# citibeth/spsparse

Hardware: NVIDIA B200
Metric: spgemm_intermediate_products_per_sec (higher is better)
Workload: dtype f64

## Files before the change

### spsparse_b200/csrc/radix_sort.cuh

```cuda
#pragma once
#include "common.cuh"

constexpr int RS_THREADS = 256;
#ifndef RS_IPT_N
#define RS_IPT_N 16
#endif
#ifndef RS_MIN_BLOCKS
#define RS_MIN_BLOCKS 3
#endif
constexpr int RS_IPT = RS_IPT_N;
constexpr int RS_HB = RS_IPT / 2;
constexpr int RS_TILE = RS_THREADS * RS_IPT;
constexpr int RS_WARPS = RS_THREADS / 32;
constexpr int RS_RADIX_BITS = 8;
constexpr int RS_RADIX = 1 << RS_RADIX_BITS;
constexpr int RS_NB = RS_RADIX + 1;
constexpr int RS_MAX_PASSES = 8;
#ifndef RS_LOOKBACK
#define RS_LOOKBACK 8
#endif
constexpr size_t RS_SMEM_BYTES =
    (size_t)RS_TILE * 16 + (size_t)RS_WARPS * RS_NB * sizeof(u32) + 64;

#define RS_WORD_AGG(c) ((c) + 1u)
// ... 72 lines not shown
    constexpr int HU = 4;
    for (u64 i0 = (u64)blockIdx.x * blockDim.x + threadIdx.x; i0 < in.n; i0 += HU * stride) {
        i32 hi[HU], lo[HU];
        double v[HU];
#pragma unroll
        for (int u = 0; u < HU; ++u) {
            const u64 i = i0 + u * stride;
            const u64 ic = i < in.n ? i : i0;
            hi[u] = ld_stream_i32(in.hi + ic);
            lo[u] = in.lo ? ld_stream_i32(in.lo + ic) : 0;
            v[u] = ld_stream_f64(in.val + ic);
        }
#pragma unroll
        for (int u = 0; u < HU; ++u) {
            const u64 i = i0 + u * stride;
            if (i >= in.n) break;
            if ((u32)hi[u] >= in.extent_hi || (u32)lo[u] >= in.extent_lo) { oob = 1; continue; }
            if (!input_kept(in, (u32)i, v[u])) continue;
            ++kept;
            u64 key = pack_key(hi[u], lo[u], in.bits_lo) >> shift0;
            for (int p = 0; p < passes; ++p) {
                atomicAdd(&s_h[p * RS_RADIX + (u32)(key & (RS_RADIX - 1))], 1u);
                key >>= RS_RADIX_BITS;
            }
        }
    }
    __syncthreads();
    for (int t = threadIdx.x; t < passes * RS_RADIX; t += blockDim.x)
        if (s_h[t]) atomicAdd(&hist[t], s_h[t]);
#pragma unroll
    for (int o = 16; o > 0; o >>= 1) kept += __shfl_xor_sync(SPB_FULL_MASK, kept, o);
    if (lane_id() == 0 && kept) atomicAdd(&counters[0], kept);
    if (oob) counters[1] = 1;
}

__global__ void __launch_bounds__(512) k_keys_hist(const u64 *__restrict__ keys, u64 n, int passes, u32 *hist) {
    __shared__ u32 s_h[RS_MAX_PASSES * RS_RADIX];
    for (int t = threadIdx.x; t < passes * RS_RADIX; t += blockDim.x) s_h[t] = 0;
    __syncthreads();
    const u64 stride = (u64)gridDim.x * blockDim.x;
    for (u64 i = (u64)blockIdx.x * blockDim.x + threadIdx.x; i < n; i += stride) {
        u64 key = ld_stream_u64(keys + i);
        for (int p = 0; p < passes; ++p) {
            atomicAdd(&s_h[p * RS_RADIX + (u32)(key & (RS_RADIX - 1))], 1u);
            key >>= RS_RADIX_BITS;
        }
    }
    __syncthreads();
    for (int t = threadIdx.x; t < passes * RS_RADIX; t += blockDim.x)
        if (s_h[t]) atomicAdd(&hist[t], s_h[t]);
}

__global__ void __launch_bounds__(RS_RADIX) k_bucket_starts(u32 *hist) {
    __shared__ u32 s_w[RS_RADIX / 32];
    u32 *h = hist + blockIdx.x * RS_RADIX;
    u32 c = h[threadIdx.x];
    u32 incl = warp_incl_scan(c);
    if (lane_id() == 31) s_w[threadIdx.x >> 5] = incl;
    __syncthreads();
    u32 add = 0;
    for (u32 w = 0; w < (threadIdx.x >> 5); ++w) add += s_w[w];
    h[threadIdx.x] = add + incl - c;
}

struct PassArgs {
    const u64 *keys_in;
    const double *vals_in;
    u64 *keys_out;
    double *vals_out;
    const u32 *n_ptr;
    const u32 *bucket_start;
    u32 *lookback;
    u32 *ticket;
    int shift;
    int rank_mode;
};

template <bool PASS0, bool BULK = false>
__global__ void __launch_bounds__(RS_THREADS, RS_MIN_BLOCKS) k_radix_pass(PassArgs a, SortInput in) {
    __shared__ __align__(8) u64 s_mbar[2];
    extern __shared__ __align__(128) unsigned char smem_raw[];
    u64 *s_keys = reinterpret_cast<u64 *>(smem_raw);
    double *s_vals = reinterpret_cast<double *>(s_keys + RS_TILE);
    u32 *s_wcnt = reinterpret_cast<u32 *>(s_vals + RS_TILE);
    u32 *s_misc = s_wcnt + RS_WARPS * RS_NB;

    const u32 tid = threadIdx.x, lane = tid & 31, warp = tid >> 5;
    if (tid == 0) {
        s_misc[0] = atomicAdd(a.ticket, 1u);
        if (BULK) { mbar_init(&s_mbar[0], 1); mbar_init(&s_mbar[1], 1); mbar_fence_init(); }
    }
    for (int t = tid; t < RS_WARPS * RS_NB; t += RS_THREADS) s_wcnt[t] = 0;
    __syncthreads();
    const u32 tile = s_misc[0];
    const u32 n = PASS0 ? in.n : *a.n_ptr;
    const u64 tile_base = (u64)tile * RS_TILE;
    if (tile_base >= n) return;
    if (BULK && PASS0 && tid == 0) {
        i32 *s_idx = reinterpret_cast<i32 *>(s_keys);
        mbar_expect_tx(&s_mbar[0], (in.lo ? 2u : 1u) * RS_TILE * 4u);
        bulk_load(s_idx, in.hi + tile_base, RS_TILE * 4u, &s_mbar[0]);
        if (in.lo) bulk_load(s_idx + RS_TILE, in.lo + tile_base, RS_TILE * 4u, &s_mbar[0]);
        mbar_expect_tx(&s_mbar[1], RS_TILE * 8u);
        bulk_load(s_vals, in.val + tile_base, RS_TILE * 8u, &s_mbar[1]);
    }
    if (BULK && !PASS0 && tid == 0) {
        const u32 valid = n - tile_base < (u64)RS_TILE ? (u32)(n - tile_base) : (u32)RS_TILE;
        const u32 bytes = (valid * 8u + 15u) & ~15u;
        mbar_expect_tx(&s_mbar[0], bytes);
        bulk_load(s_keys, a.keys_in + tile_base, bytes, &s_mbar[0]);
        mbar_expect_tx(&s_mbar[1], bytes);
        bulk_load(s_vals, a.vals_in + tile_base, bytes, &s_mbar[1]);
    }

    const u64 wbase = tile_base + (u64)warp * (32 * RS_IPT) + lane;
    u64 key[RS_IPT];
    u32 valid_bits = 0;
    if (PASS0 && BULK) {
        mbar_wait(&s_mbar[0], 0);
        mbar_wait(&s_mbar[1], 0);
        const i32 *s_idx = reinterpret_cast<const i32 *>(s_keys);
#pragma unroll
        for (int k = 0; k < RS_IPT; ++k) {
            const u32 q = warp * (32 * RS_IPT) + k * 32 + lane;
            const i32 hi = s_idx[q], lo = in.lo ? s_idx[RS_TILE + q] : 0;
            const bool ok = ((u32)hi < in.extent_hi) && ((u32)lo < in.extent_lo) && input_kept(in, (u32)(tile_base + q), s_vals[q]);
            key[k] = pack_key(hi, lo, in.bits_lo);
            valid_bits |= (ok ? 1u : 0u) << k;
        }
    } else if (PASS0) {
#pragma unroll
        for (int h = 0; h < RS_IPT; h += RS_HB) {
            i32 hi[RS_HB], lo[RS_HB];
            double v[RS_HB];
#pragma unroll
            for (int k = 0; k < RS_HB; ++k) {
                u64 i = wbase + (u64)(h + k) * 32;
                u64 ic = i < n ? i : (u64)n - 1;
                hi[k] = ld_stream_i32(in.hi + ic);
                lo[k] = in.lo ? ld_stream_i32(in.lo + ic) : 0;
                v[k] = in.val[ic];
            }
#pragma unroll
            for (int k = 0; k < RS_HB; ++k) {
                u64 i = wbase + (u64)(h + k) * 32;
                bool ok = (i < n) && ((u32)hi[k] < in.extent_hi) && ((u32)lo[k] < in.extent_lo) &&
                          input_kept(in, (u32)i, v[k]);
                key[h + k] = pack_key(hi[k], lo[k], in.bits_lo);
                valid_bits |= (ok ? 1u : 0u) << (h + k);
            }
        }
    } else if (BULK) {
        mbar_wait(&s_mbar[0], 0);
#pragma unroll
        for (int k = 0; k < RS_IPT; ++k) {
            const bool ok = wbase + (u64)k * 32 < n;
            key[k] = ok ? s_keys[warp * (32 * RS_IPT) + k * 32 + lane] : 0;
            valid_bits |= (ok ? 1u : 0u) << k;
        }
    } else {
#pragma unroll
        for (int k = 0; k < RS_IPT; ++k) {
            u64 i = wbase + (u64)k * 32;
            bool ok = i < n;
            key[k] = ok ? ld_stream_u64(a.keys_in + i) : 0;
            valid_bits |= (ok ? 1u : 0u) << k;
        }
#pragma unroll
        for (int k = 0; k < RS_IPT; ++k) {
            u64 i = wbase + (u64)k * 32;
            if (i < n && (lane & 15) == 0) asm volatile("prefetch.global.L2 [%0];" ::"l"(a.vals_in + i));
        }
    }

    u32 *mycnt = s_wcnt + warp * RS_NB;
    const u32 lt = lanemask_lt();
    unsigned short pos[RS_IPT];
#pragma unroll
    for (int k = 0; k < RS_IPT; ++k) {
        const bool ok = (valid_bits >> k) & 1u;
        const u32 d = (u32)((key[k] >> a.shift) & (RS_RADIX - 1));
        u32 peers;
        if (a.rank_mode == 0) {
            peers = __ballot_sync(SPB_FULL_MASK, ok);
#pragma unroll
            for (int b = 0; b < RS_RADIX_BITS; ++b) {
                int sgn;
                asm("bfe.s32 %0, %1, %2, 1;" : "=r"(sgn) : "r"(d), "r"(b));
                const u32 m = __ballot_sync(SPB_FULL_MASK, sgn != 0);
                peers &= ~(m ^ (u32)sgn);
            }
        } else {
            peers = __match_any_sync(SPB_FULL_MASK, ok ? d : (u32)RS_RADIX);
        }
        u32 leader = ok ? (u32)(__ffs(peers) - 1) : lane;
        u32 before = 0;
        if (ok && lane == leader) {
            before = mycnt[d];
            mycnt[d] = before + __popc(peers);
        }
        before = __shfl_sync(SPB_FULL_MASK, before, leader);
        pos[k] = (unsigned short)(before + __popc(peers & lt));
        __syncwarp();
    }
    __syncthreads();

    u32 total = 0;
#pragma unroll
    for (int w = 0; w < RS_WARPS; ++w) total += s_wcnt[w * RS_NB + tid];
    u32 *lb = a.lookback + (u64)tile * RS_RADIX + tid;
    st_relaxed_u32(lb, tile == 0 ? RS_WORD_INCL(total) : RS_WORD_AGG(total));
    u32 incl = warp_incl_scan(total);
    if (lane == 31) s_misc[1 + warp] = incl;
    __syncthreads();
    u32 lstart = incl - total;
    for (u32 w = 0; w < warp; ++w) lstart += s_misc[1 + w];
    const u32 nvalid_if_last = lstart + total;
    {
        u32 run = lstart;
#pragma unroll
        for (int w = 0; w < RS_WARPS; ++w) {
            u32 c = s_wcnt[w * RS_NB + tid];
            s_wcnt[w * RS_NB + tid] = run;
            run += c;
        }
    }
    if (tid == RS_RADIX - 1) s_misc[12] = nvalid_if_last;
    __syncthreads();
    const u32 nvalid = s_misc[12];

#pragma unroll
    for (int k = 0; k < RS_IPT; ++k) {
        if ((valid_bits >> k) & 1u) {
            u32 d = (u32)((key[k] >> a.shift) & (RS_RADIX - 1));
            u32 p = mycnt[d] + pos[k];
            pos[k] = (unsigned short)p;
            s_keys[p] = key[k];
        }
    }
    {
        const double *vsrc = PASS0 ? in.val : a.vals_in;
        double v[RS_IPT];
        if (BULK) {
            mbar_wait(&s_mbar[1], 0);
#pragma unroll
            for (int k = 0; k < RS_IPT; ++k) v[k] = s_vals[warp * (32 * RS_IPT) + k * 32 + lane];
            __syncthreads();
        } else {
#pragma unroll
            for (int k = 0; k < RS_IPT; ++k) {
                u64 i = wbase + (u64)k * 32;
                v[k] = ((valid_bits >> k) & 1u) ? ld_stream_f64(vsrc + i) : 0.0;
            }
        }
#pragma unroll
        for (int k = 0; k < RS_IPT; ++k)
            if ((valid_bits >> k) & 1u) s_vals[pos[k]] = v[k];
    }

    u32 excl = 0;
    if (tile > 0) {
        i64 p = (i64)tile - 1;
        bool done = false;
        while (!done) {
            u32 w[RS_LOOKBACK];
#pragma unroll
            for (int u = 0; u < RS_LOOKBACK; ++u)
                w[u] = (p - u >= 0) ? ld_relaxed_u32(a.lookback + (u64)(p - u) * RS_RADIX + tid) : RS_WORD_INCL(0u);
#pragma unroll
            for (int u = 0; u < RS_LOOKBACK; ++u) {
                if (done) break;
                while (!RS_READY(w[u])) w[u] = ld_relaxed_u32(a.lookback + (u64)(p - u) * RS_RADIX + tid);
                excl += RS_VALUE(w[u]);
                if (RS_IS_INCL(w[u])) done = true;
            }
            p -= RS_LOOKBACK;
        }
        st_relaxed_u32(lb, RS_WORD_INCL(excl + total));
    }
    const u32 gbase = a.bucket_start[tid] + excl - lstart;
    __syncthreads();
    s_wcnt[tid] = gbase;
    __syncthreads();

#pragma unroll
    for (int k = 0; k < RS_IPT; ++k) {
        u32 p = (u32)k * RS_THREADS + tid;
        if (p < nvalid) {
            u64 kk = s_keys[p];
            u32 dst = s_wcnt[(u32)((kk >> a.shift) & (RS_RADIX - 1))] + p;
            a.keys_out[dst] = kk;
            a.vals_out[dst] = s_vals[p];
        }
    }
}

constexpr int SG_THREADS = 256;
constexpr int SG_IPT = 8;
constexpr int SG_TILE = SG_THREADS * SG_IPT;
constexpr int SEG_MAX = 64;

constexpr int SG_CNT_SHIFT = 8;
__global__ void __launch_bounds__(SG_THREADS, 5) k_segment_sort(const u64 *__restrict__ keys_in, const double *__restrict__ vals_in,
                                                                const u32 *n_ptr, int bits_lo, u64 *keys_out, double *vals_out,
                                                                unsigned char *flags, u32 *long_count, u64 *tile_cnt = nullptr,
                                                                int keep_all = 0) {
    constexpr int W = SG_TILE + 2 * SEG_MAX;
    constexpr int ITS = (W + SG_THREADS - 1) / SG_THREADS;
    constexpr int NG = ITS * SG_THREADS / 32;
    __shared__ u64 s_key[W];
    __shared__ u32 s_col[W];
    __shared__ u32 s_hb[NG];
    __shared__ u32 s_last[NG];
    __shared__ u32 s_first[NG];
    const u32 n = *n_ptr;
    const u64 base = (u64)blockIdx.x * SG_TILE;
    if (base >= n) return;
    const u32 tid = threadIdx.x, lane = tid & 31, warp = tid >> 5;
    for (u32 q = tid; q < (u32)W; q += SG_THREADS) {
        const i64 g = (i64)base + (i64)q - SEG_MAX;
        s_key[q] = (g >= 0 && g < (i64)n) ? ld_stream_u64(keys_in + g) : ~0ull;
    }
#pragma unroll
    for (int k = 0; k < SG_IPT; ++k) {
        const u64 g = base + (u64)warp * 256 + (u64)k * 32 + lane;
        if (g < n && (lane & 15) == 0) asm volatile("prefetch.global.L2 [%0];" ::"l"(vals_in + g));
    }
    __syncthreads();
    const u64 lo_mask = (1ull << bits_lo) - 1;
#pragma unroll
    for (int it = 0; it < ITS; ++it) {
        const u32 q = (u32)it * SG_THREADS + tid;
        bool head = true;
        if (q < (u32)W) {
            const u64 kk = s_key[q];
            s_col[q] = (u32)(kk & lo_mask);
            head = q == 0 || (s_key[q - 1] >> bits_lo) != (kk >> bits_lo);
        }
        const u32 hb = __ballot_sync(SPB_FULL_MASK, head);
        if (lane == 0) {
            const u32 g = q >> 5;
            s_hb[g] = hb;
            s_last[g] = hb ? (g << 5) + 31 - __clz(hb) : 0;
            s_first[g] = hb ? (g << 5) + __ffs(hb) - 1 : 0xffffffffu;
        }
    }
    __syncthreads();
    if (warp == 0) {
        u32 carry = 0;
        for (int r = 0; r < (NG + 31) / 32; ++r) {
            const int g = r * 32 + (int)lane;
            const u32 mine = g < NG ? s_last[g] : 0;
            u32 inc = mine;
#pragma unroll
            for (int o = 1; o < 32; o <<= 1) {
                const u32 t = __shfl_up_sync(SPB_FULL_MASK, inc, o);
                if (lane >= (u32)o) inc = max(inc, t);
            }
            u32 exc = __shfl_up_sync(SPB_FULL_MASK, inc, 1);
            if (lane == 0) exc = 0;
            if (g < NG) s_last[g] = max(exc, carry);
            carry = max(carry, __shfl_sync(SPB_FULL_MASK, inc, 31));
        }
        carry = 0xffffffffu;
        for (int r = (NG + 31) / 32 - 1; r >= 0; --r) {
            const int g = r * 32 + (int)lane;
            const u32 mine = g < NG ? s_first[g] : 0xffffffffu;
            u32 inc = mine;
#pragma unroll
            for (int o = 1; o < 32; o <<= 1) {
                const u32 t = __shfl_down_sync(SPB_FULL_MASK, inc, o);
                if (lane + o < 32) inc = min(inc, t);
            }
            u32 exc = __shfl_down_sync(SPB_FULL_MASK, inc, 1);
            if (lane == 31) exc = 0xffffffffu;
            if (g < NG) s_first[g] = min(exc, carry);
            carry = min(carry, __shfl_sync(SPB_FULL_MASK, inc, 0));
        }
    }
    __syncthreads();
    u32 n_long = 0;
    i32 shift_by[SG_IPT];
    u32 cnt_at = 0, cnt_before = 0, cnt_after = 0;
    const u64 wbase = base + (u64)warp * 256;
#pragma unroll
    for (int k = 0; k < SG_IPT; ++k) {
        const u32 q = SEG_MAX + warp * 256 + (u32)k * 32 + lane;
        const u64 g = wbase + (u64)k * 32 + lane;
        shift_by[k] = 0;
        if (g < n) {
            bool head = true, rhead = false;
            const u32 grp = q >> 5, l = q & 31, hb = s_hb[grp];
            const u32 below = hb & (0xffffffffu >> (31 - l));
            const u32 st = below ? (grp << 5) + 31 - __clz(below) : s_last[grp];
            const u32 above = l < 31 ? hb & (0xffffffffu << (l + 1)) : 0u;
            const u32 nx = above ? (grp << 5) + __ffs(above) - 1 : s_first[grp];
            const bool is_long = nx - st > (u32)SEG_MAX;
            if (!is_long) {
                const u32 col = s_col[q];
                u32 before = 0, same = 0;
                for (u32 j = st; j < q; ++j) { before += s_col[j] <= col; same += s_col[j] == col; }
                for (u32 j = q + 1; j < nx; ++j) before += s_col[j] < col;
                shift_by[k] = (i32)(st + before) - (i32)q;
                head = keep_all || same == 0;
                rhead = before == 0;
            }
            if (flags) flags[g] = is_long;
            n_long += is_long;
            const u64 dst = (u64)((i64)g + shift_by[k]);
            const u32 inc = (head ? 1u : 0u) | (rhead ? 0x10000u : 0u);
            if (dst < wbase) cnt_before += inc;
            else if (dst >= wbase + 256) cnt_after += inc;
            else cnt_at += inc;
        }
    }
    if (tile_cnt) {
        const u32 a0 = __reduce_add_sync(SPB_FULL_MASK, cnt_at), a1 = __reduce_add_sync(SPB_FULL_MASK, cnt_before),
                  a2 = __reduce_add_sync(SPB_FULL_MASK, cnt_after);
        if (lane == 0) {
            u64 *t = tile_cnt + (wbase >> SG_CNT_SHIFT);
            if (a0) atomicAdd((ull *)t, (ull)(a0 & 0xffffu) | ((ull)(a0 >> 16) << 31));
            if (a1) atomicAdd((ull *)(t - 1), (ull)(a1 & 0xffffu) | ((ull)(a1 >> 16) << 31));
            if (a2) atomicAdd((ull *)(t + 1), (ull)(a2 & 0xffffu) | ((ull)(a2 >> 16) << 31));
        }
    }
    double v[SG_IPT];
#pragma unroll
    for (int k = 0; k < SG_IPT; ++k) {
        const u64 g = wbase + (u64)k * 32 + lane;
        v[k] = g < n ? ld_stream_f64(vals_in + g) : 0.0;
    }
#pragma unroll
    for (int k = 0; k < SG_IPT; ++k) {
        const u64 g = wbase + (u64)k * 32 + lane;
        if (g < n) {
            const u64 dst = (u64)((i64)g + shift_by[k]);
            keys_out[dst] = s_key[SEG_MAX + warp * 256 + k * 32 + lane];
            vals_out[dst] = v[k];
        }
    }
    n_long = __reduce_add_sync(SPB_FULL_MASK, n_long);
    if (n_long && lane == 0) atomicAdd(long_count, n_long);
}

static_assert(SG_TILE % 256 == 0 && (1 << SG_CNT_SHIFT) == 256, "a warp's 256 consecutive entries are one tile of the reduce pass");
#ifndef SGW_UNROLL_N
#define SGW_UNROLL_N 8
#endif
constexpr int SGW_UNROLL = SGW_UNROLL_N;
__global__ void __launch_bounds__(SG_THREADS, 6) k_segment_sort_walk(const u64 *__restrict__ keys_in, const double *__restrict__ vals_in,
                                                             const u32 *n_ptr, int bits_lo, u64 *keys_out, double *vals_out,
                                                             unsigned char *flags, u32 *long_count, u64 *tile_cnt = nullptr,
                                                             int keep_all = 0) {
    __shared__ u32 s_row[SG_TILE + 2 * SEG_MAX];
    __shared__ u32 s_col[SG_TILE + 2 * SEG_MAX];
    const u32 n = *n_ptr;
    const u64 base = (u64)blockIdx.x * SG_TILE;
    if (base >= n) return;
    const u32 tid = threadIdx.x;
    const u32 lo_mask = bits_lo >= 32 ? 0xffffffffu : (1u << bits_lo) - 1u;
    for (u32 q = tid; q < SG_TILE + 2 * SEG_MAX; q += SG_THREADS) {
        const i64 g = (i64)base + (i64)q - SEG_MAX;
        u32 row = 0xffffffffu, col = 0;
        if (g >= 0 && g < (i64)n) {
            const u64 key = ld_stream_u64(keys_in + g);
            row = (u32)(key >> bits_lo);
            col = (u32)key & lo_mask;
        }
        s_row[q] = row;
        s_col[q] = col;
    }
    const u32 lane = tid & 31, warp = tid >> 5;
    const u64 wbase = base + (u64)warp * 256;
    double v[SG_IPT];
#pragma unroll
    for (int k = 0; k < SG_IPT; ++k) {
        const u64 g = wbase + (u64)k * 32 + lane;
        v[k] = g < n ? ld_stream_f64(vals_in + g) : 0.0;
    }
    __syncthreads();
    u32 n_long = 0;
    u32 cnt_at = 0, cnt_before = 0, cnt_after = 0;
#pragma unroll
    for (int k = 0; k < SG_IPT; ++k) {
        const u32 q = SEG_MAX + warp * 256 + (u32)k * 32 + lane;
        const u64 g = wbase + (u64)k * 32 + lane;
        u64 dst = g;
        bool head = true, rhead = false;
        if (g < n) {
            const u32 row = s_row[q], col = s_col[q];
            u32 b = 0, f = 0, before = 0, same = 0;
            if (s_row[q - SEG_MAX] == row || s_row[q + SEG_MAX] == row) b = f = (u32)SEG_MAX;
            else {
#pragma unroll SGW_UNROLL
                for (b = 0; b < (u32)SEG_MAX; ++b) {
                    if (s_row[q - 1 - b] != row) break;
                    const u32 c = s_col[q - 1 - b];
                    before += c <= col;
                    same += c == col;
                }
#pragma unroll SGW_UNROLL
                for (f = 0; f < (u32)SEG_MAX; ++f) {
                    if (s_row[q + 1 + f] != row) break;
                    before += s_col[q + 1 + f] < col;
                }
            }
            const bool is_long = b == (u32)SEG_MAX || f == (u32)SEG_MAX || b + f + 1 > (u32)SEG_MAX;
            if (!is_long) {
                dst = g - b + before;
                head = keep_all || same == 0;
                rhead = before == 0;
            }
            keys_out[dst] = ((u64)row << bits_lo) | col;
            vals_out[dst] = v[k];
            if (flags) flags[g] = is_long;
            n_long += is_long;
            const u32 inc = (head ? 1u : 0u) | (rhead ? 0x10000u : 0u);
            if (dst < wbase) cnt_before += inc;
            else if (dst >= wbase + 256) cnt_after += inc;
            else cnt_at += inc;
        }
    }
    if (tile_cnt) {
        const u32 a0 = __reduce_add_sync(SPB_FULL_MASK, cnt_at), a1 = __reduce_add_sync(SPB_FULL_MASK, cnt_before),
                  a2 = __reduce_add_sync(SPB_FULL_MASK, cnt_after);
        if (lane == 0) {
            u64 *t = tile_cnt + (wbase >> SG_CNT_SHIFT);
            if (a0) atomicAdd((ull *)t, (ull)(a0 & 0xffffu) | ((ull)(a0 >> 16) << 31));
            if (a1) atomicAdd((ull *)(t - 1), (ull)(a1 & 0xffffu) | ((ull)(a1 >> 16) << 31));
            if (a2) atomicAdd((ull *)(t + 1), (ull)(a2 & 0xffffu) | ((ull)(a2 >> 16) << 31));
        }
    }
    n_long = __reduce_add_sync(SPB_FULL_MASK, n_long);
    if (n_long && lane == 0) atomicAdd(long_count, n_long);
}

constexpr int SGS_ROW = 5;
constexpr int SGS_H = SGS_ROW - 1;
constexpr int SGS_STEP = 32 - 2 * SGS_H;
constexpr int SGS_STEPS = (256 + SGS_STEP - 1) / SGS_STEP;
__global__ void __launch_bounds__(SG_THREADS, 6) k_segment_sort_shfl(const u64 *__restrict__ keys_in, const double *__restrict__ vals_in,
                                                                    const u32 *n_ptr, int bits_lo, u64 *keys_out, double *vals_out,
                                                                    unsigned char *flags, u32 *long_count, u64 *tile_cnt = nullptr,
                                                                    int keep_all = 0) {
    __shared__ u32 s_row[SG_TILE + 2 * SEG_MAX];
    __shared__ u32 s_col[SG_TILE + 2 * SEG_MAX];
    __shared__ double s_val[SG_TILE];
    const u32 n = *n_ptr;
    const u64 base = (u64)blockIdx.x * SG_TILE;
    if (base >= n) return;
    const u32 tid = threadIdx.x, lane = tid & 31, warp = tid >> 5;
    const u32 lo_mask = bits_lo >= 32 ? 0xffffffffu : (1u << bits_lo) - 1u;
    for (u32 q = tid; q < SG_TILE + 2 * SEG_MAX; q += SG_THREADS) {
        const i64 g = (i64)base + (i64)q - SEG_MAX;
        u32 row = 0xffffffffu, col = 0;
        if (g >= 0 && g < (i64)n) {
            const u64 key = ld_stream_u64(keys_in + g);
            row = (u32)(key >> bits_lo);
            col = (u32)key & lo_mask;
        }
        s_row[q] = row;
        s_col[q] = col;
    }
#pragma unroll
    for (int k = 0; k < SG_IPT; ++k) {
        const u32 e = (u32)k * SG_THREADS + tid;
        const u64 g = base + e;
        s_val[e] = g < n ? ld_stream_f64(vals_in + g) : 0.0;
    }
    __syncthreads();
    const u64 wbase = base + (u64)warp * 256;
    u32 n_long = 0;
    u32 cnt_at = 0, cnt_before = 0, cnt_after = 0;
    for (int t = 0; t < SGS_STEPS; ++t) {
        const i32 e = t * SGS_STEP + (i32)lane - SGS_H;
        const u32 q = (u32)(SEG_MAX + (i32)warp * 256 + e);
        const u64 g = wbase + (u64)(i64)e;
        const bool mine = lane >= (u32)SGS_H && lane < (u32)(32 - SGS_H) && e < 256 && g < n;
        const u32 row = s_row[q], col = s_col[q];
        const u32 hb = __ballot_sync(SPB_FULL_MASK, s_row[q - 1] != row);
        const u32 tail = __shfl_sync(SPB_FULL_MASK, (u32)(s_row[q + 1] != row), 31);
        const u64 z = ~((u64)hb | ((u64)tail << 32)) & 0x1ffffffffull;
        u64 run = z;
#pragma unroll
        for (int d = 1; d < SGS_ROW; ++d) run &= z >> d;
        u32 b = 0, f = 0, before = 0, same = 0;
        if (run == 0) {
#pragma unroll
            for (int d = 1; d < SGS_ROW; ++d) {
                const u32 ru = __shfl_up_sync(SPB_FULL_MASK, row, d), cu = __shfl_up_sync(SPB_FULL_MASK, col, d);
                const u32 rd = __shfl_down_sync(SPB_FULL_MASK, row, d), cd = __shfl_down_sync(SPB_FULL_MASK, col, d);
                const bool up = lane >= (u32)d && ru == row, dn = lane + d < 32u && rd == row;
                b += up;
                before += (up && cu <= col) + (dn && cd < col);
                same += up && cu == col;
                f += dn;
            }
        } else if (mine) {
            if (s_row[q - SEG_MAX] == row || s_row[q + SEG_MAX] == row) b = f = (u32)SEG_MAX;
            else {
                for (b = 0; b < (u32)SEG_MAX; ++b) {
                    if (s_row[q - 1 - b] != row) break;
                    const u32 c = s_col[q - 1 - b];
                    before += c <= col;
                    same += c == col;
                }
                for (f = 0; f < (u32)SEG_MAX; ++f) {
                    if (s_row[q + 1 + f] != row) break;
                    before += s_col[q + 1 + f] < col;
                }
            }
        }
        if (mine) {
            const bool is_long = b == (u32)SEG_MAX || f == (u32)SEG_MAX || b + f + 1 > (u32)SEG_MAX;
            u64 dst = g;
            bool head = true, rhead = false;
            if (!is_long) {
                dst = g - b + before;
                head = keep_all || same == 0;
                rhead = before == 0;
            }
            keys_out[dst] = ((u64)row << bits_lo) | col;
            vals_out[dst] = s_val[warp * 256 + (u32)e];
            if (flags) flags[g] = is_long;
            n_long += is_long;
            const u32 inc = (head ? 1u : 0u) | (rhead ? 0x10000u : 0u);
            if (dst < wbase) cnt_before += inc;
            else if (dst >= wbase + 256) cnt_after += inc;
            else cnt_at += inc;
        }
    }
    if (tile_cnt) {
        const u32 a0 = __reduce_add_sync(SPB_FULL_MASK, cnt_at), a1 = __reduce_add_sync(SPB_FULL_MASK, cnt_before),
                  a2 = __reduce_add_sync(SPB_FULL_MASK, cnt_after);
        if (lane == 0) {
            u64 *t = tile_cnt + (wbase >> SG_CNT_SHIFT);
            if (a0) atomicAdd((ull *)t, (ull)(a0 & 0xffffu) | ((ull)(a0 >> 16) << 31));
            if (a1) atomicAdd((ull *)(t - 1), (ull)(a1 & 0xffffu) | ((ull)(a1 >> 16) << 31));
            if (a2) atomicAdd((ull *)(t + 1), (ull)(a2 & 0xffffu) | ((ull)(a2 >> 16) << 31));
        }
    }
    n_long = __reduce_add_sync(SPB_FULL_MASK, n_long);
    if (n_long && lane == 0) atomicAdd(long_count, n_long);
}

__global__ void k_gather_flagged(const u64 *__restrict__ keys, const double *__restrict__ vals, const unsigned char *__restrict__ flags,
                                 const u64 *__restrict__ slot, u32 n, u64 *k_out, double *v_out) {
    for (u64 e = (u64)blockIdx.x * blockDim.x + threadIdx.x; e < n; e += (u64)gridDim.x * blockDim.x)
        if (flags[e]) { k_out[slot[e]] = keys[e]; v_out[slot[e]] = vals[e]; }
}
__global__ void k_scatter_flagged(const u64 *__restrict__ k_sorted, const double *__restrict__ v_sorted,
                                  const unsigned char *__restrict__ flags, const u64 *__restrict__ slot, u32 n, u64 *keys, double *vals) {
    for (u64 e = (u64)blockIdx.x * blockDim.x + threadIdx.x; e < n; e += (u64)gridDim.x * blockDim.x)
        if (flags[e]) { keys[e] = k_sorted[slot[e]]; vals[e] = v_sorted[slot[e]]; }
}
```

### spsparse_b200/csrc/reduce_by_key.cuh

```cuda
#pragma once
#include "scan.cuh"

#ifndef RK_THREADS_N
#define RK_THREADS_N 256
#endif
constexpr int RK_THREADS = RK_THREADS_N;
constexpr int RK_IPT = 8;
constexpr int RK_TILE = RK_THREADS * RK_IPT;
constexpr int RK_WARPS = RK_THREADS / 32;
constexpr u32 RK_LONG_RUN = 256;

enum { POLICY_LEAVE_ALONE = 0, POLICY_ADD = 1, POLICY_REPLACE = 2, POLICY_KEEP_ALL = 3 };
enum { MODE_CONSOLIDATE = 0, MODE_ESC = 1 };

struct ReduceArgs {
    const u64 *keys;
    const double *vals;
    const u32 *n_ptr;
    int bits_lo;
    int policy;
    i32 *out_hi;
    i32 *out_lo;
    double *out_val;
    u32 *out_count;
    u64 *state;
    u32 *ticket;
    u32 *long_list;
    u32 *long_count;
    u32 long_cap;
    u32 *row_start;
    i32 *row_id;
    u32 *row_count;
    const i32 *row_ids;
    i32 row_base;
    const double *si;
    const double *sk;
    double C;
};

__device__ __forceinline__ u32 rk_phys(u32 L) { return L + (L >> 3); }
constexpr int RK_SLOTS = RK_TILE + 2 + ((RK_TILE + 2) >> 3) + 1;

#ifndef RK_MIN_BLOCKS
#define RK_MIN_BLOCKS 5
#endif
template <int MODE>
__global__ void __launch_bounds__(RK_THREADS, RK_MIN_BLOCKS) k_reduce_by_key(ReduceArgs a) {
    __shared__ u64 s_keys[RK_SLOTS];
    __shared__ double s_vals[RK_SLOTS];
    __shared__ u64 s_warp[RK_WARPS];
    __shared__ u32 s_tile;
    __shared__ u64 s_excl;
    const u32 tid = threadIdx.x, lane = tid & 31, warp = tid >> 5;
    const bool want_rows = (MODE == MODE_CONSOLIDATE) && (a.row_start != nullptr);
    if (tid == 0) s_tile = atomicAdd(a.ticket, 1u);
    __syncthreads();
    const u32 tile = s_tile;
    const u32 n = *a.n_ptr;
    const u64 base = (u64)tile * RK_TILE;
    if (base >= n) return;
    const u32 tile_n = (n - base < (u64)RK_TILE) ? (u32)(n - base) : (u32)RK_TILE;

#pragma unroll
    for (int k = 0; k < RK_IPT; ++k) {
        u32 p = (u32)k * RK_THREADS + tid;
        if (p < tile_n) {
            s_keys[rk_phys(p + 1)] = ld_stream_u64(a.keys + base + p);
            s_vals[rk_phys(p + 1)] = ld_stream_f64(a.vals + base + p);
        }
    }
    if (tid == 0) s_keys[0] = base ? a.keys[base - 1] : 0;
    if (tid == 32 && base + RK_TILE < n) s_keys[rk_phys(RK_TILE + 1)] = a.keys[base + RK_TILE];
    __syncthreads();

    const u32 first = tid * RK_IPT;
    const u32 mine = first < tile_n ? (tile_n - first < (u32)RK_IPT ? tile_n - first : (u32)RK_IPT) : 0;
    u64 key[RK_IPT];
    double acc[RK_IPT];
    u32 head_bits = 0, rhead_bits = 0, defer_bits = 0;
    if (mine) {
        u64 prev = s_keys[rk_phys(first)];
#pragma unroll
        for (int j = 0; j < RK_IPT; ++j) {
            key[j] = s_keys[rk_phys(first + j + 1)];
            acc[j] = s_vals[rk_phys(first + j + 1)];
        }
        int cur = -1;
#pragma unroll
        for (int j = 0; j < RK_IPT; ++j) {
            if ((u32)j < mine) {
                const u64 before = j ? key[j - 1] : prev;
                const bool head = (a.policy == POLICY_KEEP_ALL) || (base + first + j == 0) || (key[j] != before);
                if (head) {
                    head_bits |= 1u << j;
                    if (want_rows && ((base + first + j == 0) || (key[j] >> a.bits_lo) != (before >> a.bits_lo)))
                        rhead_bits |= 1u << j;
                    cur = j;
                } else if (cur >= 0) {
                    double v = acc[j];
#pragma unroll
                    for (int h = 0; h < RK_IPT; ++h)
                        if (h == cur) {
                            if (a.policy == POLICY_ADD) acc[h] = __dadd_rn(acc[h], v);
                            else if (a.policy == POLICY_REPLACE) acc[h] = v;
                        }
                }
            }
        }
        if (cur >= 0 && mine == (u32)RK_IPT && (a.policy == POLICY_ADD || a.policy == POLICY_REPLACE)) {
            const u64 k0 = key[RK_IPT - 1];
            double sum = 0.0;
#pragma unroll
            for (int h = 0; h < RK_IPT; ++h) if (h == cur) sum = acc[h];
            u64 q = base + first + RK_IPT;
            u32 steps = 0;
            while (q < n) {
                const u32 L = (u32)(q - base) + 1;
                u64 kq;
                double vq = 0.0;
                if (L <= (u32)RK_TILE) { kq = s_keys[rk_phys(L)]; vq = s_vals[rk_phys(L)]; }
                else if (L == (u32)RK_TILE + 1) { kq = s_keys[rk_phys(L)]; if (kq == k0) vq = a.vals[q]; }
                else { kq = a.keys[q]; if (kq == k0) vq = a.vals[q]; }
                if (kq != k0) break;
                if (a.policy == POLICY_ADD) sum = __dadd_rn(sum, vq); else sum = vq;
                ++q;
                if (MODE == MODE_CONSOLIDATE && ++steps >= RK_LONG_RUN) { defer_bits |= 1u << cur; break; }
            }
#pragma unroll
            for (int h = 0; h < RK_IPT; ++h) if (h == cur) acc[h] = sum;
        }
    }
    u32 emit_bits = head_bits;
    if (MODE == MODE_ESC) {
        const u64 lo_mask = (1ull << a.bits_lo) - 1;
#pragma unroll
        for (int j = 0; j < RK_IPT; ++j)
            if ((head_bits >> j) & 1u) {
                const u32 kcol = (u32)(key[j] & lo_mask);
                if (acc[j] == 0.0 || (a.sk && a.sk[kcol] == 0.0)) emit_bits &= ~(1u << j);
            }
    }
    const u64 my = (u64)__popc(emit_bits) | ((u64)__popc(rhead_bits) << 32);
    const u64 incl = warp_incl_scan(my);
    if (lane == 31) s_warp[warp] = incl;
    __syncthreads();
    u64 wbefore = 0, total = 0;
#pragma unroll
    for (int w = 0; w < RK_WARPS; ++w) {
        const u64 t = s_warp[w];
        if ((u32)w < warp) wbefore += t;
        total += t;
    }
    const u64 before_me = wbefore + incl - my;
    const u32 tile_out = (u32)(total & 0xffffffffull);
    if (warp == 0) {
        const u64 packed = (total & 0xffffffffull) | ((total >> 32) << 31);
        const u64 excl0 = lookback_exclusive(a.state, tile, packed);
        if (lane == 0) {
            s_excl = excl0;
            if (base + RK_TILE >= n) {
                const u64 fin = excl0 + packed;
                const u32 n_out = (u32)(fin & 0x7fffffffull), n_rows = (u32)(fin >> 31);
                *a.out_count = n_out;
                if (want_rows) { *a.row_count = n_rows; a.row_start[n_rows] = n_out; }
            }
        }
    }
    {
        u32 slot = (u32)(before_me & 0xffffffffull);
#pragma unroll
        for (int j = 0; j < RK_IPT; ++j) {
            if ((emit_bits >> j) & 1u) {
                double v = acc[j];
                if (MODE == MODE_ESC) {
                    const u64 lo_mask = (1ull << a.bits_lo) - 1;
                    const i32 hi = (i32)(key[j] >> a.bits_lo) + a.row_base;
                    v = __dmul_rn(v, a.C);
                    v = __dmul_rn(v, a.si ? a.si[a.row_ids[hi]] : 1.0);
                    v = __dmul_rn(v, a.sk ? a.sk[(u32)(key[j] & lo_mask)] : 1.0);
                }
                s_keys[slot] = key[j];
                s_vals[slot] = v;
                ++slot;
            }
        }
    }
    __syncthreads();
    const u64 excl_rows = s_excl >> 31;
    const u64 excl = s_excl & 0x7fffffffull;
    if (MODE == MODE_CONSOLIDATE && (rhead_bits | defer_bits)) {
        u32 slot = (u32)(before_me & 0xffffffffull);
        u64 rslot = excl_rows + (before_me >> 32);
#pragma unroll
        for (int j = 0; j < RK_IPT; ++j) {
            if ((emit_bits >> j) & 1u) {
                if ((rhead_bits >> j) & 1u) {
                    a.row_start[rslot] = (u32)(excl + slot);
                    a.row_id[rslot] = (i32)(key[j] >> a.bits_lo);
                    ++rslot;
                }
                if ((defer_bits >> j) & 1u) {
                    u32 t = atomicAdd(a.long_count, 1u);
                    if (t < a.long_cap) { a.long_list[2 * t] = (u32)(excl + slot); a.long_list[2 * t + 1] = (u32)(base + first + j); }
                }
                ++slot;
            }
        }
    }
    const u64 lo_mask = (1ull << a.bits_lo) - 1;
    for (u32 t = tid; t < tile_out; t += RK_THREADS) {
        const u64 k = s_keys[t];
        i32 hi = (i32)(k >> a.bits_lo);
        if (MODE == MODE_ESC) hi += a.row_base;
        a.out_hi[excl + t] = hi;
        if (a.out_lo) a.out_lo[excl + t] = (i32)(k & lo_mask);
        a.out_val[excl + t] = s_vals[t];
    }
}

__global__ void __launch_bounds__(256) k_long_runs(ReduceArgs a) {
    const u32 n = *a.n_ptr;
    u32 cnt = *a.long_count;
    if (cnt > a.long_cap) cnt = a.long_cap;
    const u32 lane = lane_id();
    const u32 warps = gridDim.x * (blockDim.x >> 5);
    for (u32 t = blockIdx.x * (blockDim.x >> 5) + (threadIdx.x >> 5); t < cnt; t += warps) {
        const u32 slot = a.long_list[2 * t], start = a.long_list[2 * t + 1];
        const u64 key = a.keys[start];
        u32 lo = start + 1, step = RK_LONG_RUN;
        u32 hi = n;
        for (;;) {
            const u64 probe = (u64)lo + step;
            if (probe >= n) break;
            if (a.keys[probe] > key) { hi = (u32)probe; break; }
            lo = (u32)probe + 1;
            step *= 2;
        }
        while (lo < hi) {
            const u32 mid = lo + (hi - lo) / 2;
            if (a.keys[mid] <= key) lo = mid + 1; else hi = mid;
        }
        const u32 end = lo;
        double r;
        if (a.policy == POLICY_ADD) {
            double sum = 0.0;
            bool first = true;
            u32 i = start;
            double v = (i + lane < end) ? a.vals[i + lane] : 0.0;
            while (i < end) {
                const u32 m = end - i < 32u ? end - i : 32u;
                const u32 inext = i + 32;
                const double vn = (inext < end && inext + lane < end) ? a.vals[inext + lane] : 0.0;
                for (u32 l = 0; l < m; ++l) {
                    const double x = __shfl_sync(SPB_FULL_MASK, v, (int)l);
                    if (first) { sum = x; first = false; }
                    else sum = __dadd_rn(sum, x);
                }
                v = vn;
                i = inext;
            }
            r = sum;
        } else {
            r = (a.policy == POLICY_REPLACE) ? a.vals[end - 1] : a.vals[start];
        }
        if (lane == 0) a.out_val[slot] = r;
    }
}
```

### spsparse_b200/csrc/reduce_segsort.cuh

```cuda
#pragma once
#include "radix_sort.cuh"
#include "reduce_by_key.cuh"

constexpr int RF_H = SEG_MAX;
constexpr int RF_W = RK_TILE + 2 * RF_H;
constexpr int RF_ITS = (RF_W + RK_THREADS - 1) / RK_THREADS;
constexpr int RF_SORTED = RK_TILE + RF_H + 1;
constexpr int RF_SLOTS = RF_SORTED + (RF_SORTED >> 3) + 1;

struct RfSmem {
    u64 raw[RF_W];
    u64 keys[RF_SLOTS];
    double vals[RF_SLOTS];
    u64 warp[RK_WARPS];
    u64 excl;
    u32 tile;
};

__global__ void __launch_bounds__(RK_THREADS, 4) k_reduce_segsort(ReduceArgs a, u32 *seg_long) {
    extern __shared__ __align__(16) unsigned char rf_smem[];
    RfSmem &s = *reinterpret_cast<RfSmem *>(rf_smem);
    const u32 tid = threadIdx.x, lane = tid & 31, warp = tid >> 5;
    const bool want_rows = a.row_start != nullptr;
    if (tid == 0) s.tile = atomicAdd(a.ticket, 1u);
    __syncthreads();
    const u32 tile = s.tile;
    const u32 n = *a.n_ptr;
    const u64 base = (u64)tile * RK_TILE;
    if (base >= n) return;
    const u32 tile_n = (n - base < (u64)RK_TILE) ? (u32)(n - base) : (u32)RK_TILE;

    double v[RF_ITS];
#pragma unroll
    for (int k = 0; k < RF_ITS; ++k) {
        const u32 q = (u32)k * RK_THREADS + tid;
        const i64 g = (i64)base + (i64)q - RF_H;
        const bool in = q < (u32)RF_W && g >= 0 && g < (i64)n;
        if (q < (u32)RF_W) s.raw[q] = in ? ld_stream_u64(a.keys + g) : ~0ull;
        v[k] = in ? ld_stream_f64(a.vals + g) : 0.0;
    }
    __syncthreads();

    const u64 lo_mask = (1ull << a.bits_lo) - 1;
    u32 n_long = 0;
#pragma unroll
    for (int k = 0; k < RF_ITS; ++k) {
        const u32 q = (u32)k * RK_THREADS + tid;
        if (q >= (u32)RF_W) continue;
        const u64 key = s.raw[q];
        if (key == ~0ull) continue;
        const u64 row = key >> a.bits_lo, col = key & lo_mask;
        u32 b = 0, f = 0, before = 0;
        bool cut = false;
        for (; b < (u32)SEG_MAX; ++b) {
            if (q < 1 + b) { cut = true; break; }
            const u64 kk = s.raw[q - 1 - b];
            if ((kk >> a.bits_lo) != row) break;
            before += (kk & lo_mask) <= col;
        }
        for (; f < (u32)SEG_MAX; ++f) {
            if (q + 1 + f >= (u32)RF_W) { cut = true; break; }
            const u64 kk = s.raw[q + 1 + f];
            if ((kk >> a.bits_lo) != row) break;
            before += (kk & lo_mask) < col;
        }
        const bool is_long = b == (u32)SEG_MAX || f == (u32)SEG_MAX || b + f + 1 > (u32)SEG_MAX;
        if (q >= (u32)RF_H && q < (u32)(RF_H + RK_TILE)) n_long += is_long;
        const u32 place = (cut || is_long) ? q : q - b + before;
        if (place + 1 >= (u32)RF_H && place + 1 < (u32)(RF_H + RF_SORTED)) {
            const u32 L = place + 1 - (u32)RF_H;
            s.keys[rk_phys(L)] = key;
            s.vals[rk_phys(L)] = v[k];
        }
    }
    n_long = __reduce_add_sync(SPB_FULL_MASK, n_long);
    if (n_long && lane == 0) atomicAdd(seg_long, n_long);
    __syncthreads();

    const u32 first = tid * RK_IPT;
    const u32 mine = first < tile_n ? (tile_n - first < (u32)RK_IPT ? tile_n - first : (u32)RK_IPT) : 0;
    u64 key[RK_IPT];
    double acc[RK_IPT];
    u32 head_bits = 0, rhead_bits = 0;
    if (mine) {
        const u64 prev = s.keys[rk_phys(first)];
#pragma unroll
        for (int j = 0; j < RK_IPT; ++j) {
            key[j] = s.keys[rk_phys(first + j + 1)];
            acc[j] = s.vals[rk_phys(first + j + 1)];
        }
        int cur = -1;
#pragma unroll
        for (int j = 0; j < RK_IPT; ++j) {
            if ((u32)j < mine) {
                const u64 before = j ? key[j - 1] : prev;
                const bool head = (a.policy == POLICY_KEEP_ALL) || (base + first + j == 0) || (key[j] != before);
                if (head) {
                    head_bits |= 1u << j;
                    if (want_rows && ((base + first + j == 0) || (key[j] >> a.bits_lo) != (before >> a.bits_lo)))
                        rhead_bits |= 1u << j;
                    cur = j;
                } else if (cur >= 0) {
                    const double vj = acc[j];
#pragma unroll
                    for (int h = 0; h < RK_IPT; ++h)
                        if (h == cur) {
                            if (a.policy == POLICY_ADD) acc[h] = __dadd_rn(acc[h], vj);
                            else if (a.policy == POLICY_REPLACE) acc[h] = vj;
                        }
                }
            }
        }
        if (cur >= 0 && mine == (u32)RK_IPT && (a.policy == POLICY_ADD || a.policy == POLICY_REPLACE)) {
            const u64 k0 = key[RK_IPT - 1];
            double sum = 0.0;
#pragma unroll
            for (int h = 0; h < RK_IPT; ++h) if (h == cur) sum = acc[h];
            u64 q = base + first + RK_IPT;
            while (q < n) {
                const u32 L = (u32)(q - base) + 1;
                if (L >= (u32)RF_SORTED) break;
                if (s.keys[rk_phys(L)] != k0) break;
                const double vq = s.vals[rk_phys(L)];
                if (a.policy == POLICY_ADD) sum = __dadd_rn(sum, vq); else sum = vq;
                ++q;
            }
#pragma unroll
            for (int h = 0; h < RK_IPT; ++h) if (h == cur) acc[h] = sum;
        }
    }
    const u32 emit_bits = head_bits;
    const u64 my = (u64)__popc(emit_bits) | ((u64)__popc(rhead_bits) << 32);
    const u64 incl = warp_incl_scan(my);
    if (lane == 31) s.warp[warp] = incl;
    __syncthreads();
    u64 wbefore = 0, total = 0;
#pragma unroll
    for (int w = 0; w < RK_WARPS; ++w) {
        const u64 t = s.warp[w];
        if ((u32)w < warp) wbefore += t;
        total += t;
    }
    const u64 before_me = wbefore + incl - my;
    const u32 tile_out = (u32)(total & 0xffffffffull);
    if (warp == 0) {
        const u64 packed = (total & 0xffffffffull) | ((total >> 32) << 31);
        const u64 excl0 = lookback_exclusive(a.state, tile, packed);
        if (lane == 0) {
            s.excl = excl0;
            if (base + RK_TILE >= n) {
                const u64 fin = excl0 + packed;
                const u32 n_out = (u32)(fin & 0x7fffffffull), n_rows = (u32)(fin >> 31);
                *a.out_count = n_out;
                if (want_rows) { *a.row_count = n_rows; a.row_start[n_rows] = n_out; }
            }
        }
    }
    {
        u32 slot = (u32)(before_me & 0xffffffffull);
#pragma unroll
        for (int j = 0; j < RK_IPT; ++j) {
            if ((emit_bits >> j) & 1u) {
                s.keys[slot] = key[j];
                s.vals[slot] = acc[j];
                ++slot;
            }
        }
    }
    __syncthreads();
    const u64 excl_rows = s.excl >> 31;
    const u64 excl = s.excl & 0x7fffffffull;
    if (rhead_bits) {
        u32 slot = (u32)(before_me & 0xffffffffull);
        u64 rslot = excl_rows + (before_me >> 32);
#pragma unroll
        for (int j = 0; j < RK_IPT; ++j) {
            if ((emit_bits >> j) & 1u) {
                if ((rhead_bits >> j) & 1u) {
                    a.row_start[rslot] = (u32)(excl + slot);
                    a.row_id[rslot] = (i32)(key[j] >> a.bits_lo);
                    ++rslot;
                }
                ++slot;
            }
        }
    }
    for (u32 t = tid; t < tile_out; t += RK_THREADS) {
        const u64 k = s.keys[t];
        a.out_hi[excl + t] = (i32)(k >> a.bits_lo);
        if (a.out_lo) a.out_lo[excl + t] = (i32)(k & lo_mask);
        a.out_val[excl + t] = s.vals[t];
    }
}
```

### spsparse_b200/csrc/reduce_warp.cuh

```cuda
#pragma once
#include "reduce_by_key.cuh"

constexpr int RW_IPT = 8;
constexpr int RW_TILE = 32 * RW_IPT;
constexpr int RW_WARPS = 8;
constexpr int RW_THREADS = 32 * RW_WARPS;
constexpr int RW_SLOTS = RW_TILE + (RW_TILE >> 3) + 1;
#ifndef RW_MIN_BLOCKS
#define RW_MIN_BLOCKS 4
#endif

template <bool LOOKBACK>
__global__ void __launch_bounds__(RW_THREADS, RW_MIN_BLOCKS) k_reduce_warp(ReduceArgs a) {
    __shared__ u64 s_keys[RW_WARPS][RW_SLOTS];
    __shared__ double s_vals[RW_WARPS][RW_SLOTS];
    __shared__ u32 s_ticket;
    const u32 tid = threadIdx.x, lane = tid & 31, warp = tid >> 5;
    u32 tile = blockIdx.x * RW_WARPS + warp;
    if (LOOKBACK) {
        if (tid == 0) s_ticket = atomicAdd(a.ticket, 1u);
        __syncthreads();
        tile = s_ticket * RW_WARPS + warp;
    }
    const u32 n = *a.n_ptr;
    const u64 base = (u64)tile * RW_TILE;
    if (base >= n) return;
    const u32 tile_n = (n - base < (u64)RW_TILE) ? (u32)(n - base) : (u32)RW_TILE;
    const bool want_rows = a.row_start != nullptr;
    const u32 first = lane * RW_IPT;
    const u32 mine = first < tile_n ? (tile_n - first < (u32)RW_IPT ? tile_n - first : (u32)RW_IPT) : 0;

    u64 key[RW_IPT];
    double acc[RW_IPT];
    if (tile_n == (u32)RW_TILE && ((((uintptr_t)a.keys) | ((uintptr_t)a.vals)) & 15u) == 0) {
        const ulonglong2 *kp = reinterpret_cast<const ulonglong2 *>(a.keys + base + first);
        const double2 *vp = reinterpret_cast<const double2 *>(a.vals + base + first);
#pragma unroll
        for (int j = 0; j < RW_IPT / 2; ++j) {
            const ulonglong2 t = __ldg(kp + j);
            key[2 * j] = t.x; key[2 * j + 1] = t.y;
        }
#pragma unroll
        for (int j = 0; j < RW_IPT / 2; ++j) {
            const double2 t = __ldg(vp + j);
            acc[2 * j] = t.x; acc[2 * j + 1] = t.y;
        }
    } else {
#pragma unroll
        for (int j = 0; j < RW_IPT; ++j) {
            key[j] = 0; acc[j] = 0.0;
            if ((u32)j < mine) { key[j] = a.keys[base + first + j]; acc[j] = a.vals[base + first + j]; }
        }
    }
    u64 prev = __shfl_up_sync(SPB_FULL_MASK, key[RW_IPT - 1], 1);
    if (lane == 0) prev = base ? a.keys[base - 1] : 0;
    u64 next = __shfl_down_sync(SPB_FULL_MASK, key[0], 1);
    const bool more = base + first + RW_IPT < n;
    if (lane == 31 && more) next = a.keys[base + RW_TILE];

    u32 head_bits = 0, rhead_bits = 0, defer_bits = 0;
    if (mine) {
        int cur = -1;
#pragma unroll
        for (int j = 0; j < RW_IPT; ++j) {
            if ((u32)j < mine) {
                const u64 before = j ? key[j - 1] : prev;
                const bool head = (a.policy == POLICY_KEEP_ALL) || (base + first + j == 0) || (key[j] != before);
                if (head) {
                    head_bits |= 1u << j;
                    if (want_rows && ((base + first + j == 0) || (key[j] >> a.bits_lo) != (before >> a.bits_lo)))
                        rhead_bits |= 1u << j;
                    cur = j;
                } else if (cur >= 0) {
                    const double v = acc[j];
#pragma unroll
                    for (int h = 0; h < RW_IPT; ++h)
                        if (h == cur) {
                            if (a.policy == POLICY_ADD) acc[h] = __dadd_rn(acc[h], v);
                            else if (a.policy == POLICY_REPLACE) acc[h] = v;
                        }
                }
            }
        }
        if (cur >= 0 && mine == (u32)RW_IPT && more && next == key[RW_IPT - 1] &&
            (a.policy == POLICY_ADD || a.policy == POLICY_REPLACE)) {
            const u64 k0 = key[RW_IPT - 1];
            double sum = 0.0;
#pragma unroll
            for (int h = 0; h < RW_IPT; ++h) if (h == cur) sum = acc[h];
            u64 q = base + first + RW_IPT;
            u32 steps = 0;
            while (q < n) {
                if (a.keys[q] != k0) break;
                const double vq = a.vals[q];
                if (a.policy == POLICY_ADD) sum = __dadd_rn(sum, vq); else sum = vq;
                ++q;
                if (++steps >= RK_LONG_RUN) { defer_bits |= 1u << cur; break; }
            }
#pragma unroll
            for (int h = 0; h < RW_IPT; ++h) if (h == cur) acc[h] = sum;
        }
    }
    const u32 emit_bits = head_bits;
    const u64 my = (u64)__popc(emit_bits) | ((u64)__popc(rhead_bits) << 32);
    const u64 incl = warp_incl_scan(my);
    const u64 total = __shfl_sync(SPB_FULL_MASK, incl, 31);
    const u64 before_me = incl - my;
    const u32 tile_out = (u32)(total & 0xffffffffull);
    const u64 packed = (total & 0xffffffffull) | ((total >> 32) << 31);
    const u64 excl0 = LOOKBACK ? lookback_exclusive(a.state, tile, packed) : a.state[tile];
    if (lane == 0 && base + RW_TILE >= n) {
        const u64 fin = excl0 + packed;
        const u32 n_out = (u32)(fin & 0x7fffffffull), n_rows = (u32)(fin >> 31);
        *a.out_count = n_out;
        if (want_rows) { *a.row_count = n_rows; a.row_start[n_rows] = n_out; }
    }
    const u64 excl_rows = excl0 >> 31;
    const u64 excl = excl0 & 0x7fffffffull;
    u64 *const sk = s_keys[warp];
    double *const sv = s_vals[warp];
    {
        u32 slot = (u32)(before_me & 0xffffffffull);
        u64 rslot = excl_rows + (before_me >> 32);
#pragma unroll
        for (int j = 0; j < RW_IPT; ++j) {
            if ((emit_bits >> j) & 1u) {
                sk[rk_phys(slot)] = key[j];
                sv[rk_phys(slot)] = acc[j];
                if ((rhead_bits >> j) & 1u) {
                    a.row_start[rslot] = (u32)(excl + slot);
                    a.row_id[rslot] = (i32)(key[j] >> a.bits_lo);
                    ++rslot;
                }
                if ((defer_bits >> j) & 1u) {
                    const u32 t = atomicAdd(a.long_count, 1u);
                    if (t < a.long_cap) { a.long_list[2 * t] = (u32)(excl + slot); a.long_list[2 * t + 1] = (u32)(base + first + j); }
                }
                ++slot;
            }
        }
    }
    __syncwarp();
    const u64 lo_mask = (1ull << a.bits_lo) - 1;
    for (u32 t = lane; t < tile_out; t += 32) {
        const u64 k = sk[rk_phys(t)];
        a.out_hi[excl + t] = (i32)(k >> a.bits_lo);
        if (a.out_lo) a.out_lo[excl + t] = (i32)(k & lo_mask);
        a.out_val[excl + t] = sv[rk_phys(t)];
    }
}
```

### spsparse_b200/csrc/spb_api.cu

```cuda
#include "../../include/spsparse_b200.h"

#include <cstdarg>
#include <cstdio>
#include <cstdlib>
#include <cstring>
#include <chrono>
#include <map>
#include <mutex>
#include <thread>
#include <unordered_map>
#include <vector>

#include "common.cuh"
#include "csr.cuh"
#include "gen.cuh"
#include "radix_sort.cuh"
#include "radix_sort9.cuh"
#include "reduce_by_key.cuh"
#include "reduce_segsort.cuh"
#include "reduce_warp.cuh"
#include "scan.cuh"
#include "spgemm.cuh"
#include "dense_ops.cuh"
#include "rowpart.cuh"

thread_local std::string g_last_error;

int spb_fail(int code, const char *fmt, ...) {
    char buf[1024];
    va_list ap;
    va_start(ap, fmt);
    vsnprintf(buf, sizeof buf, fmt, ap);
    va_end(ap);
    g_last_error = buf;
    return code;
}

static inline double now_ms() {
    return std::chrono::duration<double, std::milli>(std::chrono::steady_clock::now().time_since_epoch()).count();
}
static double g_alloc_ms = 0;
static int g_trace = -1;
static inline bool tracing() {
    if (g_trace < 0) g_trace = getenv("SPB_TRACE") ? 1 : 0;
    return g_trace == 1;
}

struct DevPool {
    std::multimap<size_t, void *> free_;
    std::unordered_map<void *, size_t> live_;
    std::mutex mu_;
    size_t cached_bytes = 0;

    static size_t round_up(size_t b) {
        if (b < 512) return 512;
        if (b < (1u << 20)) return (b + 511) & ~(size_t)511;
        return (b + (1u << 20) - 1) & ~(size_t)((1u << 20) - 1);
    }
    cudaError_t alloc(void **out, size_t bytes) {
        std::lock_guard<std::mutex> g(mu_);
        const size_t want = round_up(bytes);
        auto it = free_.lower_bound(want);
        if (it != free_.end() && it->first <= want + (want >= (64u << 20) ? want / 2 : want / 8)) {
            *out = it->second;
            live_[*out] = it->first;
            cached_bytes -= it->first;
            free_.erase(it);
            return cudaSuccess;
        }
        void *p = nullptr;
        cudaError_t e = cudaMalloc(&p, want);
        if (e != cudaSuccess) {
            cudaGetLastError();
            trim_locked();
            e = cudaMalloc(&p, want);
            if (e != cudaSuccess) return e;
        }
        live_[p] = want;
        *out = p;
        return cudaSuccess;
    }
    void release(void *p) {
        if (!p) return;
        std::lock_guard<std::mutex> g(mu_);
        auto it = live_.find(p);
        if (it == live_.end()) return;
        free_.insert({it->second, p});
        cached_bytes += it->second;
        live_.erase(it);
    }
    void trim_locked() {
        cudaDeviceSynchronize();
        for (auto &kv : free_) cudaFree(kv.second);
        free_.clear();
        cached_bytes = 0;
    }
    void destroy() {
        std::lock_guard<std::mutex> g(mu_);
        trim_locked();
        for (auto &kv : live_) cudaFree(kv.first);
        live_.clear();
    }
};

struct spb_ctx {
    int device;
    cudaStream_t stream;
    bool own_stream;
    int sm_count;
    u32 merge_max_products;
    u64 esc_chunk;
    u64 hash_min_products;
    int hash_variant;
    u64 launches;
    bool bulk_load;
    static constexpr int XFER_WORKERS = 8;
    int xfer_workers;
    static constexpr size_t XFER_CHUNK = 16u << 20;
    void *xfer_buf[XFER_WORKERS][2];
    cudaStream_t xfer_stream[XFER_WORKERS];
    cudaEvent_t xfer_ev[XFER_WORKERS][2];
    bool xfer_ready;
    DevPool pool;
};

struct spb_coo {
    int rank;
    u64 shape[2];
    u64 n;
    i32 *idx[2];
    double *val;
    int sort_order[2];
    bool owned;
    u32 *row_start;
    i32 *row_id;
    u32 nrows;
    bool rows_valid;
    u32 *dense_ptr;
    bool dense_ptr_owned;
    u32 *range_ptr;
    u64 range_lo, range_hi;
    u32 max_row_len;
};

struct Scratch {
    spb_ctx *ctx;
    std::vector<void *> ptrs;
    explicit Scratch(spb_ctx *c) : ctx(c) {}
    ~Scratch() { for (void *p : ptrs) ctx->pool.release(p); }
    template <typename T>
    int get(T **out, u64 count) {
        void *p = nullptr;
        size_t bytes = (size_t)(count ? count : 1) * sizeof(T);
        double t0 = tracing() ? now_ms() : 0;
        cudaError_t e = ctx->pool.alloc(&p, bytes);
        if (tracing()) { double dt = now_ms() - t0; g_alloc_ms += dt; if (dt > 1.0) fprintf(stderr, "[spb] pool.alloc(%zu MB) took %.2f ms\n", bytes >> 20, dt); }
        if (e != cudaSuccess) return spb_fail(SPB_ERR_CUDA, "device allocation of %zu bytes failed: %s", bytes, cudaGetErrorString(e));
        ptrs.push_back(p);
        *out = (T *)p;
        return 0;
    }
    template <typename T>
    int zeroed(T **out, u64 count) {
        CKR(get(out, count));
        CK(cudaMemsetAsync(*out, 0, (size_t)(count ? count : 1) * sizeof(T), ctx->stream));
        return 0;
    }
    void release(void *p) {
        for (size_t i = 0; i < ptrs.size(); ++i)
            if (ptrs[i] == p) { ctx->pool.release(p); ptrs.erase(ptrs.begin() + i); return; }
    }
    void keep(void *p) {
        for (size_t i = 0; i < ptrs.size(); ++i)
            if (ptrs[i] == p) { ptrs.erase(ptrs.begin() + i); return; }
    }
};

struct Timer {
    cudaStream_t s;
    std::vector<cudaEvent_t> ev;
    explicit Timer(cudaStream_t st) : s(st) {}
    ~Timer() { for (auto e : ev) cudaEventDestroy(e); }
    int mark() {
        cudaEvent_t e;
        cudaEventCreate(&e);
        cudaEventRecord(e, s);
        ev.push_back(e);
        return (int)ev.size() - 1;
    }
    float ms(int a, int b) {
        float t = 0;
        cudaEventSynchronize(ev[b]);
        cudaEventElapsedTime(&t, ev[a], ev[b]);
        return t;
    }
};

static inline u32 grid_for(u64 n, u32 threads, u32 cap) {
    u64 g = div_up(n ? n : 1, threads);
    return (u32)(g < cap ? g : cap);
}

static bool host_ptr_is_pinned(const void *p) {
    cudaPointerAttributes at;
    if (cudaPointerGetAttributes(&at, p) != cudaSuccess) { cudaGetLastError(); return false; }
    return at.type == cudaMemoryTypeHost || at.type == cudaMemoryTypeManaged;
}

static int xfer_setup(spb_ctx *c) {
    if (c->xfer_ready) return 0;
    {
        int want = getenv("SPB_XFER_WORKERS") ? atoi(getenv("SPB_XFER_WORKERS")) : (int)(std::thread::hardware_concurrency() / 2);
        c->xfer_workers = want < 1 ? 1 : (want > spb_ctx::XFER_WORKERS ? spb_ctx::XFER_WORKERS : want);
    }
    for (int w = 0; w < c->xfer_workers; ++w) {
        CK(cudaStreamCreateWithFlags(&c->xfer_stream[w], cudaStreamNonBlocking));
        for (int b = 0; b < 2; ++b) {
            CK(cudaHostAlloc(&c->xfer_buf[w][b], spb_ctx::XFER_CHUNK, cudaHostAllocDefault));
            CK(cudaEventCreateWithFlags(&c->xfer_ev[w][b], cudaEventDisableTiming));
        }
    }
    c->xfer_ready = true;
    return 0;
}

struct XferJob { void *dev; void *host; size_t bytes; };

static int staged_copy(spb_ctx *c, const XferJob *jobs, int njobs, bool to_device) {
    bool all_pinned = true;
    size_t total = 0;
    for (int j = 0; j < njobs; ++j) { if (jobs[j].bytes) { all_pinned = all_pinned && host_ptr_is_pinned(jobs[j].host); total += jobs[j].bytes; } }
    if (all_pinned || total < (4u << 20)) {
        for (int j = 0; j < njobs; ++j)
            if (jobs[j].bytes)
                CK(cudaMemcpyAsync(to_device ? jobs[j].dev : jobs[j].host, to_device ? jobs[j].host : jobs[j].dev, jobs[j].bytes,
                                   to_device ? cudaMemcpyHostToDevice : cudaMemcpyDeviceToHost, c->stream));
        CK(cudaStreamSynchronize(c->stream));
        return 0;
    }
    CKR(xfer_setup(c));
    struct Chunk { char *dev; char *host; size_t bytes; };
    std::vector<Chunk> chunks;
    for (int j = 0; j < njobs; ++j)
        for (size_t o = 0; o < jobs[j].bytes; o += spb_ctx::XFER_CHUNK)
            chunks.push_back({(char *)jobs[j].dev + o, (char *)jobs[j].host + o, std::min(spb_ctx::XFER_CHUNK, jobs[j].bytes - o)});
    const int NW = c->xfer_workers;
    cudaError_t err[spb_ctx::XFER_WORKERS];
    auto work = [&](int w) {
        cudaError_t e = cudaSetDevice(c->device);
        int b = 0;
        size_t pending_chunk[2] = {(size_t)-1, (size_t)-1};
        for (size_t k = w; k < chunks.size() && e == cudaSuccess; k += (size_t)NW, b ^= 1) {
            const Chunk &ch = chunks[k];
            if (to_device) {
                e = cudaEventSynchronize(c->xfer_ev[w][b]);
                if (e != cudaSuccess) break;
                memcpy(c->xfer_buf[w][b], ch.host, ch.bytes);
                e = cudaMemcpyAsync(ch.dev, c->xfer_buf[w][b], ch.bytes, cudaMemcpyHostToDevice, c->xfer_stream[w]);
                if (e == cudaSuccess) e = cudaEventRecord(c->xfer_ev[w][b], c->xfer_stream[w]);
            } else {
                e = cudaMemcpyAsync(c->xfer_buf[w][b], ch.dev, ch.bytes, cudaMemcpyDeviceToHost, c->xfer_stream[w]);
                if (e == cudaSuccess) e = cudaEventRecord(c->xfer_ev[w][b], c->xfer_stream[w]);
                pending_chunk[b] = k;
                const int o = b ^ 1;
                if (e == cudaSuccess && pending_chunk[o] != (size_t)-1) {
                    e = cudaEventSynchronize(c->xfer_ev[w][o]);
                    if (e == cudaSuccess) memcpy(chunks[pending_chunk[o]].host, c->xfer_buf[w][o], chunks[pending_chunk[o]].bytes);
                    pending_chunk[o] = (size_t)-1;
                }
            }
        }
        if (!to_device)
            for (int o = 0; o < 2 && e == cudaSuccess; ++o)
                if (pending_chunk[o] != (size_t)-1) {
                    e = cudaEventSynchronize(c->xfer_ev[w][o]);
                    if (e == cudaSuccess) memcpy(chunks[pending_chunk[o]].host, c->xfer_buf[w][o], chunks[pending_chunk[o]].bytes);
                }
        if (e == cudaSuccess) e = cudaStreamSynchronize(c->xfer_stream[w]);
        err[w] = e;
    };
    CK(cudaStreamSynchronize(c->stream));
    std::thread th[spb_ctx::XFER_WORKERS];
    for (int w = 1; w < NW; ++w) th[w] = std::thread(work, w);
    work(0);
    for (int w = 1; w < NW; ++w) th[w].join();
    for (int w = 0; w < NW; ++w)
        if (err[w] != cudaSuccess) return spb_fail(SPB_ERR_CUDA, "host transfer failed: %s", cudaGetErrorString(err[w]));
    return 0;
}

extern "C" {

const char *spb_last_error(void) { return g_last_error.c_str(); }
int spb_version(void) { return 100; }

int spb_ctx_create(int device, void *cuda_stream, spb_ctx **out) {
    if (!out) return spb_fail(SPB_ERR_ARG, "spb_ctx_create: out is null");
    int count = 0;
    cudaError_t e = cudaGetDeviceCount(&count);
    if (e != cudaSuccess || count == 0)
        return spb_fail(SPB_ERR_CUDA, "no CUDA device available (%s); spsparse_b200 has no CPU fallback",
                        cudaGetErrorString(e));
    if (device < 0 || device >= count) return spb_fail(SPB_ERR_ARG, "device %d out of range (%d devices)", device, count);
    CK(cudaSetDevice(device));
    struct Undo {
        spb_ctx *c;
        ~Undo() {
            if (!c) return;
            if (c->own_stream && c->stream) cudaStreamDestroy(c->stream);
            delete c;
        }
    } undo{new spb_ctx()};
    spb_ctx *c = undo.c;
    c->device = device;
    c->stream = nullptr;
    c->own_stream = (cuda_stream == nullptr);
    if (c->own_stream) CK(cudaStreamCreateWithFlags(&c->stream, cudaStreamNonBlocking));
    else c->stream = (cudaStream_t)cuda_stream;
    CK(cudaDeviceGetAttribute(&c->sm_count, cudaDevAttrMultiProcessorCount, device));
    CK(cudaFuncSetAttribute(k_radix_pass<true>, cudaFuncAttributeMaxDynamicSharedMemorySize, (int)RS_SMEM_BYTES));
    CK(cudaFuncSetAttribute(k_radix_pass<false>, cudaFuncAttributeMaxDynamicSharedMemorySize, (int)RS_SMEM_BYTES));
    CK(cudaFuncSetAttribute(k_reduce_segsort, cudaFuncAttributeMaxDynamicSharedMemorySize, (int)sizeof(RfSmem)));
    CK(cudaFuncSetAttribute(k_radix_pass9<true>, cudaFuncAttributeMaxDynamicSharedMemorySize, (int)R9_SMEM_BYTES));
    CK(cudaFuncSetAttribute(k_radix_pass9<false>, cudaFuncAttributeMaxDynamicSharedMemorySize, (int)R9_SMEM_BYTES));
    CK(cudaFuncSetAttribute(k_radix_pass<false, true>, cudaFuncAttributeMaxDynamicSharedMemorySize, (int)RS_SMEM_BYTES));
    CK(cudaFuncSetAttribute(k_radix_pass<true, true>, cudaFuncAttributeMaxDynamicSharedMemorySize, (int)RS_SMEM_BYTES));
    CK(cudaFuncSetAttribute(k_radix_pass9<true, true>, cudaFuncAttributeMaxDynamicSharedMemorySize, (int)R9_SMEM_BYTES));
    CK(cudaFuncSetAttribute(k_radix_pass9<false, true>, cudaFuncAttributeMaxDynamicSharedMemorySize, (int)R9_SMEM_BYTES));
    c->bulk_load = getenv("SPB_BULK_LOAD") ? atoi(getenv("SPB_BULK_LOAD")) != 0 : true;
    const char *s = getenv("SPB_MERGE_MAX_PRODUCTS");
    c->merge_max_products = s ? (u32)strtoul(s, nullptr, 10) : 1024u;
    s = getenv("SPB_ESC_CHUNK");
    c->esc_chunk = s ? strtoull(s, nullptr, 10) : (1ull << 27);
    c->launches = 0;
    c->xfer_ready = false;
    s = getenv("SPB_HASH_MIN_PRODUCTS");
    c->hash_min_products = s ? (strcmp(s, "off") == 0 ? ~0ull : strtoull(s, nullptr, 10)) : 512ull;
    s = getenv("SPB_HASH_VARIANT");
    c->hash_variant = s ? atoi(s) : 2;
    CK(cudaFuncSetAttribute(k_hash_symbolic, cudaFuncAttributeMaxDynamicSharedMemorySize, (int)(HASH_MAX_COLS / 8)));
    CK(cudaFuncSetAttribute(k_hash_numeric<1024, 10240, 16384>, cudaFuncAttributeMaxDynamicSharedMemorySize, (int)sizeof(HashSmem<1024, 10240, 16384>)));
    CK(cudaFuncSetAttribute(k_hash_numeric<512, 5120, 8192>, cudaFuncAttributeMaxDynamicSharedMemorySize, (int)sizeof(HashSmem<512, 5120, 8192>)));
    CK(cudaFuncSetAttribute(k_hash_numeric<256, 2560, 4096>, cudaFuncAttributeMaxDynamicSharedMemorySize, (int)sizeof(HashSmem<256, 2560, 4096>)));
    if (c->esc_chunk < 1) c->esc_chunk = 1;
    undo.c = nullptr;
    *out = c;
    return SPB_OK;
}

int spb_ctx_destroy(spb_ctx *ctx) {
    if (!ctx) return SPB_OK;
    cudaSetDevice(ctx->device);
    cudaStreamSynchronize(ctx->stream);
    if (ctx->xfer_ready)
        for (int w = 0; w < ctx->xfer_workers; ++w) {
            cudaStreamDestroy(ctx->xfer_stream[w]);
            for (int b = 0; b < 2; ++b) { cudaFreeHost(ctx->xfer_buf[w][b]); cudaEventDestroy(ctx->xfer_ev[w][b]); }
        }
    ctx->pool.destroy();
    if (ctx->own_stream) cudaStreamDestroy(ctx->stream);
    delete ctx;
    return SPB_OK;
}

int spb_ctx_sync(spb_ctx *ctx) {
    if (!ctx) return spb_fail(SPB_ERR_ARG, "null context");
    CK(cudaStreamSynchronize(ctx->stream));
    return SPB_OK;
}

int spb_ctx_trim(spb_ctx *ctx, uint64_t *released_bytes) {
    if (!ctx) return spb_fail(SPB_ERR_ARG, "null context");
    CK(cudaSetDevice(ctx->device));
    std::lock_guard<std::mutex> g(ctx->pool.mu_);
    if (released_bytes) *released_bytes = ctx->pool.cached_bytes;
    ctx->pool.trim_locked();
    return SPB_OK;
}

int spb_host_prefault(void *p, uint64_t bytes) {
    if (!p || !bytes) return SPB_OK;
    unsigned nt = std::thread::hardware_concurrency();
    if (nt > 16) nt = 16;
    if (bytes < (64ull << 20) || nt < 2) nt = 1;
    constexpr uint64_t PAGE = 4096;
    auto work = [=](unsigned t) {
        volatile char *c = static_cast<volatile char *>(p);
        const uint64_t a = bytes * t / nt, b = bytes * (t + 1) / nt;
        if (a < b) c[a] = 0;
        const uint64_t base = reinterpret_cast<uintptr_t>(p);
        for (uint64_t o = ((base + a + PAGE - 1) & ~(PAGE - 1)) - base; o < b; o += PAGE) c[o] = 0;
    };
    if (nt == 1) { work(0); return SPB_OK; }
    std::vector<std::thread> th;
    for (unsigned t = 1; t < nt; ++t) th.emplace_back(work, t);
    work(0);
    for (auto &x : th) x.join();
    return SPB_OK;
}

int spb_ctx_launch_count(const spb_ctx *ctx, uint64_t *launches) {
    if (!ctx || !launches) return spb_fail(SPB_ERR_ARG, "null argument");
    *launches = ctx->launches;
    return SPB_OK;
}

int spb_ctx_device(const spb_ctx *ctx, int *device, void **cuda_stream) {
    if (!ctx) return spb_fail(SPB_ERR_ARG, "null context");
    if (device) *device = ctx->device;
    if (cuda_stream) *cuda_stream = (void *)ctx->stream;
    return SPB_OK;
}

static int coo_new(spb_ctx *ctx, int rank, const u64 *shape, u64 n, bool allocate, spb_coo **out) {
    if (!ctx || !out || !shape) return spb_fail(SPB_ERR_ARG, "null argument");
    if (rank != 1 && rank != 2) return spb_fail(SPB_ERR_ARG, "rank must be 1 or 2 (got %d)", rank);
    for (int k = 0; k < rank; ++k)
        if (shape[k] > (1ull << 31)) return spb_fail(SPB_ERR_ARG, "extent %llu exceeds the int32 index range", (ull)shape[k]);
    if (n >= (1ull << 31)) return spb_fail(SPB_ERR_TOO_LARGE, "%llu entries: the reference's own cap is 2^31 (algorithm.hpp:419)", (ull)n);
    spb_coo *a = new spb_coo();
    a->rank = rank;
    a->shape[0] = shape[0];
    a->shape[1] = rank > 1 ? shape[1] : 1;
    a->n = n;
    a->idx[0] = a->idx[1] = nullptr;
    a->val = nullptr;
    a->sort_order[0] = -1;
    a->sort_order[1] = 0;
    a->owned = allocate;
    a->row_start = nullptr;
    a->row_id = nullptr;
    a->nrows = 0;
    a->rows_valid = false;
    a->dense_ptr = nullptr;
    a->dense_ptr_owned = true;
    a->range_ptr = nullptr;
    a->range_lo = a->range_hi = 0;
    a->max_row_len = 0;
    if (allocate) {
        size_t cnt = n ? n : 1;
        cudaError_t e = cudaSetDevice(ctx->device);
        for (int k = 0; k < rank && e == cudaSuccess; ++k) e = ctx->pool.alloc((void **)&a->idx[k], cnt * sizeof(i32));
        if (e == cudaSuccess) e = ctx->pool.alloc((void **)&a->val, cnt * sizeof(double));
        if (e != cudaSuccess) {
            for (int k = 0; k < 2; ++k) ctx->pool.release(a->idx[k]);
            ctx->pool.release(a->val);
            delete a;
            return spb_fail(SPB_ERR_CUDA, "device allocation for %llu entries failed: %s", (ull)n, cudaGetErrorString(e));
        }
    }
    *out = a;
    return SPB_OK;
}

static void drop_row_cache(spb_ctx *ctx, spb_coo *a) {
    if (ctx) {
        ctx->pool.release(a->row_start);
        ctx->pool.release(a->row_id);
        if (a->dense_ptr_owned) ctx->pool.release(a->dense_ptr);
        ctx->pool.release(a->range_ptr);
    }
    a->row_start = nullptr; a->row_id = nullptr; a->dense_ptr = nullptr; a->range_ptr = nullptr;
    a->rows_valid = false; a->nrows = 0; a->max_row_len = 0;
}

static void set_order(spb_coo *a, const int *so) {
    a->sort_order[0] = -1;
    a->sort_order[1] = 0;
    if (so && so[0] >= 0) {
        a->sort_order[0] = so[0];
        a->sort_order[1] = a->rank > 1 ? so[1] : 0;
    }
}

int spb_coo_alloc(spb_ctx *ctx, int rank, const uint64_t *shape, uint64_t n, spb_coo **out) {
    return coo_new(ctx, rank, shape, n, true, out);
}

int spb_coo_upload(spb_ctx *ctx, int rank, const uint64_t *shape, const int32_t *const *idx, const double *val,
                   uint64_t n, const int *sort_order, spb_coo **out) {
    if (n && (!idx || !val)) return spb_fail(SPB_ERR_ARG, "null data pointer");
    CKR(coo_new(ctx, rank, shape, n, true, out));
    spb_coo *a = *out;
    set_order(a, sort_order);
    XferJob jobs[3];
    int nj = 0;
    for (int k = 0; k < rank && n; ++k) {
        if (!idx[k]) { spb_coo_free(ctx, a); *out = nullptr; return spb_fail(SPB_ERR_ARG, "null index pointer for dimension %d", k); }
        jobs[nj++] = {a->idx[k], const_cast<int32_t *>(idx[k]), (size_t)n * sizeof(i32)};
    }
    if (n) jobs[nj++] = {a->val, const_cast<double *>(val), (size_t)n * sizeof(double)};
    const int rc = nj ? staged_copy(ctx, jobs, nj, true) : 0;
    if (rc) {
        spb_coo_free(ctx, a);
        *out = nullptr;
        return rc;
    }
    return SPB_OK;
}

int spb_coo_wrap_device(spb_ctx *ctx, int rank, const uint64_t *shape, int32_t *const *d_idx, double *d_val,
                        uint64_t n, const int *sort_order, spb_coo **out) {
    if (n && (!d_idx || !d_val)) return spb_fail(SPB_ERR_ARG, "null device pointer");
    CKR(coo_new(ctx, rank, shape, n, false, out));
    spb_coo *a = *out;
    for (int k = 0; k < rank; ++k) a->idx[k] = d_idx ? d_idx[k] : nullptr;
    a->val = d_val;
    set_order(a, sort_order);
    return SPB_OK;
}

int spb_coo_info(const spb_coo *a, int *rank, uint64_t *shape, uint64_t *n, int *sort_order) {
    if (!a) return spb_fail(SPB_ERR_ARG, "null array");
    if (rank) *rank = a->rank;
    for (int k = 0; k < a->rank; ++k) {
        if (shape) shape[k] = a->shape[k];
        if (sort_order) sort_order[k] = a->sort_order[k];
    }
    if (n) *n = a->n;
    return SPB_OK;
}

int spb_coo_device_ptrs(const spb_coo *a, int32_t **d_idx, double **d_val) {
    if (!a) return spb_fail(SPB_ERR_ARG, "null array");
    for (int k = 0; k < a->rank; ++k) if (d_idx) d_idx[k] = a->idx[k];
    if (d_val) *d_val = a->val;
    return SPB_OK;
}

int spb_coo_set_sorted(spb_coo *a, const int *sort_order) {
    if (!a) return spb_fail(SPB_ERR_ARG, "null array");
    if (a->rows_valid || a->dense_ptr)
        return spb_fail(SPB_ERR_ARG, "spb_coo_set_sorted: the array's row structure is already in use");
    set_order(a, sort_order);
    return SPB_OK;
}

int spb_coo_download(spb_ctx *ctx, const spb_coo *a, int32_t *const *idx, double *val) {
    if (!ctx || !a) return spb_fail(SPB_ERR_ARG, "null argument");
    CK(cudaSetDevice(ctx->device));
    XferJob jobs[3];
    int nj = 0;
    if (a->n) {
        for (int k = 0; k < a->rank; ++k)
            if (idx && idx[k]) jobs[nj++] = {a->idx[k], idx[k], (size_t)a->n * sizeof(i32)};
        if (val) jobs[nj++] = {a->val, val, (size_t)a->n * sizeof(double)};
    }
    if (nj) return staged_copy(ctx, jobs, nj, false);
    CK(cudaStreamSynchronize(ctx->stream));
    return SPB_OK;
}

int spb_coo_free(spb_ctx *ctx, spb_coo *a) {
    if (!a) return SPB_OK;
    if (a->owned && ctx) {
        for (int k = 0; k < 2; ++k) if (a->idx[k]) ctx->pool.release(a->idx[k]);
        if (a->val) ctx->pool.release(a->val);
    }
    drop_row_cache(ctx, a);
    delete a;
    return SPB_OK;
}

}

struct SortJob {
    SortInput in;
    int bits_hi;
    int policy;
};

template <typename InT, typename OutT>
static int exclusive_scan(spb_ctx *ctx, Scratch &ws, const InT *in, OutT *out, u64 n);

static int run_radix_passes(spb_ctx *ctx, Scratch &ws, int first_pass, int passes, u32 n_cap, const u32 *n_ptr,
                            u32 *hist, u64 *kA, double *vA, u64 *kB, double *vB, const SortInput *in0,
                            u64 **keys_sorted, double **vals_sorted, Timer *tm, int *mark_after_first, int shift0 = 0,
                            int digit_bits = RS_RADIX_BITS) {
    const u32 tiles = (u32)div_up(n_cap ? n_cap : 1, RS_TILE);
    const bool nine = digit_bits == R9_BITS;
    const u64 radix = nine ? R9_RADIX : RS_RADIX;
    u32 *lookback, *tickets;
    CKR(ws.zeroed(&lookback, (u64)passes * tiles * radix));
    CKR(ws.zeroed(&tickets, (u64)passes));
    u64 *kin = kA, *kout = kB;
    double *vin = vA, *vout = vB;
    for (int p = 0; p < passes; ++p) {
        PassArgs a;
        a.n_ptr = n_ptr;
        a.bucket_start = hist + (u64)p * radix;
        a.lookback = lookback + (u64)p * tiles * radix;
        a.ticket = tickets + p;
        a.shift = shift0 + p * digit_bits;
        a.rank_mode = getenv("SPB_RANK_MODE") ? atoi(getenv("SPB_RANK_MODE")) : 0;
        if (p == 0 && first_pass == 0) {
            a.keys_in = nullptr; a.vals_in = nullptr; a.keys_out = kA; a.vals_out = vA;
            const bool aligned = ((((uintptr_t)in0->hi) | ((uintptr_t)in0->lo) | ((uintptr_t)in0->val)) & 15u) == 0;
            const u32 tiles_bulk = (ctx->bulk_load && aligned) ? n_cap / RS_TILE : 0;
            if (tiles_bulk) {
                ++ctx->launches;
                if (nine) k_radix_pass9<true, true><<<tiles_bulk, RS_THREADS, R9_SMEM_BYTES, ctx->stream>>>(a, *in0);
                else k_radix_pass<true, true><<<tiles_bulk, RS_THREADS, RS_SMEM_BYTES, ctx->stream>>>(a, *in0);
            }
            if (tiles > tiles_bulk) {
                ++ctx->launches;
                if (nine) k_radix_pass9<true><<<tiles - tiles_bulk, RS_THREADS, R9_SMEM_BYTES, ctx->stream>>>(a, *in0);
                else k_radix_pass<true><<<tiles - tiles_bulk, RS_THREADS, RS_SMEM_BYTES, ctx->stream>>>(a, *in0);
            }
            kin = kA; vin = vA; kout = kB; vout = vB;
            if (tm) *mark_after_first = tm->mark();
        } else {
            a.keys_in = kin; a.vals_in = vin; a.keys_out = kout; a.vals_out = vout;
            SortInput dummy;
            memset(&dummy, 0, sizeof dummy);
            ++ctx->launches;
            if (ctx->bulk_load) {
                if (nine) k_radix_pass9<false, true><<<tiles, RS_THREADS, R9_SMEM_BYTES, ctx->stream>>>(a, dummy);
                else k_radix_pass<false, true><<<tiles, RS_THREADS, RS_SMEM_BYTES, ctx->stream>>>(a, dummy);
            } else {
                if (nine) k_radix_pass9<false><<<tiles, RS_THREADS, R9_SMEM_BYTES, ctx->stream>>>(a, dummy);
                else k_radix_pass<false><<<tiles, RS_THREADS, RS_SMEM_BYTES, ctx->stream>>>(a, dummy);
            }
            u64 *tk = kin; kin = kout; kout = tk;
            double *tv = vin; vin = vout; vout = tv;
        }
    }
    CK(cudaGetLastError());
    *keys_sorted = kin;
    *vals_sorted = vin;
    return 0;
}

static int sort_reduce(spb_ctx *ctx, const SortJob &job, i32 *out_hi, i32 *out_lo, double *out_val,
                       u32 *h_kept, u32 *h_out, spb_consolidate_stats *st, u32 *row_start = nullptr,
                       i32 *row_id = nullptr, u32 *h_rows = nullptr) {
    const SortInput &in = job.in;
    const u32 n = in.n;
    const int key_bits = job.bits_hi + in.bits_lo;
    int passes_full = (key_bits + RS_RADIX_BITS - 1) / RS_RADIX_BITS;
    if (passes_full < 1) passes_full = 1;
    if (passes_full > RS_MAX_PASSES) return spb_fail(SPB_ERR_ARG, "key of %d bits is too wide", key_bits);
    int passes_row = (job.bits_hi + RS_RADIX_BITS - 1) / RS_RADIX_BITS;
    if (passes_row < 1) passes_row = 1;
    const char *seg_env = getenv("SPB_SEGMENT_SORT");
    const bool seg_short = (double)n <= 16.0 * (double)in.extent_hi && n >= (1u << 23);
    const char *walk_env = getenv("SPB_SEGMENT_WALK");
    const bool seg_walk = walk_env ? atoi(walk_env) != 0 : (double)n <= 6.0 * (double)in.extent_hi;
    const bool seg_shfl = walk_env && atoi(walk_env) == 2;
    const bool seg = in.bits_lo > 0 && passes_full - passes_row >= 2 &&
                     (seg_env ? atoi(seg_env) != 0 : seg_short);
    const int cover_bits = seg ? job.bits_hi : key_bits;
    const char *r9_env = getenv("SPB_RADIX9");
    const int passes8 = seg ? passes_row : passes_full;
    const int passes9 = cover_bits > 0 ? (cover_bits + R9_BITS - 1) / R9_BITS : 1;
    const bool nine_wanted = r9_env ? atoi(r9_env) != 0 : (seg && !seg_env);
    const bool nine = nine_wanted && passes9 < passes8;
    const int digit_bits = nine ? R9_BITS : RS_RADIX_BITS;
    const int passes = nine ? passes9 : passes8;
    const int shift0 = seg ? in.bits_lo : 0;
    if (n >= (1u << 31)) return spb_fail(SPB_ERR_TOO_LARGE, "%u entries: one sort holds fewer than 2^31 (the reference's own cap, algorithm.hpp:419)", n);
    Scratch ws(ctx);
    Timer tm(ctx->stream);
    const int t0 = tm.mark();

    u32 *hist, *counters;
    u64 *first_kept;
    CKR(ws.zeroed(&hist, (u64)passes * (nine ? R9_RADIX : RS_RADIX)));
    CKR(ws.zeroed(&counters, 8));
    CKR(ws.get(&first_kept, 2));
    CK(cudaMemsetAsync(first_kept, 0xFF, 2 * sizeof(u64), ctx->stream));
    SortInput in0 = in;
    in0.first_kept = first_kept;
    const u32 sgrid = (u32)ctx->sm_count * 4;
    if (in.drop_nan) {
        ++ctx->launches, k_first_kept_key<<<grid_for(n, 256, sgrid * 2), 256, 0, ctx->stream>>>(in0, first_kept);
        ++ctx->launches, k_first_kept_pos<<<grid_for(n, 256, sgrid * 2), 256, 0, ctx->stream>>>(in0, first_kept);
    }
    const bool vec4 = ((((uintptr_t)in0.hi) | ((uintptr_t)in0.lo) | ((uintptr_t)in0.val)) & 15u) == 0 && n >= 4096 &&
                      !(getenv("SPB_VEC_LOAD") && atoi(getenv("SPB_VEC_LOAD")) == 0);
    if (nine) {
        ++ctx->launches;
        if (vec4) k_sort_hist_v4<9><<<grid_for(n / 4, 512, sgrid), 512, 0, ctx->stream>>>(in0, passes, shift0, hist, counters);
        else k_sort_hist9<<<grid_for(n, 512, sgrid), 512, 0, ctx->stream>>>(in0, passes, shift0, hist, counters);
        ++ctx->launches, k_bucket_starts9<<<passes, R9_RADIX / 2, 0, ctx->stream>>>(hist);
    } else {
        ++ctx->launches;
        if (vec4) k_sort_hist_v4<8><<<grid_for(n / 4, 512, sgrid), 512, 0, ctx->stream>>>(in0, passes, shift0, hist, counters);
        else k_sort_hist<<<grid_for(n, 512, sgrid), 512, 0, ctx->stream>>>(in0, passes, shift0, hist, counters);
        ++ctx->launches, k_bucket_starts<<<passes, RS_RADIX, 0, ctx->stream>>>(hist);
    }
    CK(cudaGetLastError());

    u64 *kA, *kB = nullptr, *ks;
    double *vA, *vB = nullptr, *vs;
    CKR(ws.get(&kA, n));
    CKR(ws.get(&vA, n));
    if (passes > 1 || seg) { CKR(ws.get(&kB, n)); CKR(ws.get(&vB, n)); }
    int t_p0 = t0;
    CKR(run_radix_passes(ctx, ws, 0, passes, n, counters, hist, kA, vA, kB, vB, &in0, &ks, &vs, &tm, &t_p0, shift0, digit_bits));
    const int t_passes = tm.mark();
    const char *fused_env = getenv("SPB_FUSED_REDUCE");
    bool fused = seg && seg_walk && fused_env && atoi(fused_env) != 0;
    u32 h[6];
    int t1 = t_passes, t2 = t_passes;
    u64 *const ks_rows = ks;
    double *const vs_rows = vs;
    bool long_rows_fixed = false;
    const int rw_mode = getenv("SPB_REDUCE_WARP") ? atoi(getenv("SPB_REDUCE_WARP")) : 1;
    const u32 wtiles = (u32)div_up(div_up(n ? n : 1, RW_TILE), RW_WARPS) * RW_WARPS;
    for (int attempt = 0;; ++attempt) {
        ks = ks_rows; vs = vs_rows;
        u64 *ko = (ks == kA) ? kB : kA;
        double *vo = (vs == vA) ? vB : vA;
        const u32 stiles = (u32)div_up(n, SG_TILE);
        u64 *tile_off = nullptr;
        if (seg && !fused) {
            if (!long_rows_fixed) {
                u64 *tile_cnt = nullptr;
                if (rw_mode == 1) {
                    CKR(ws.zeroed(&tile_cnt, (u64)wtiles + 2));
                    CKR(ws.get(&tile_off, (u64)wtiles + 2));
                }
                const int keep_all = job.policy == POLICY_KEEP_ALL;
                ++ctx->launches;
                if (seg_shfl) k_segment_sort_shfl<<<stiles, SG_THREADS, 0, ctx->stream>>>(ks, vs, counters, in.bits_lo, ko, vo, nullptr, counters + 5, tile_cnt, keep_all);
                else if (seg_walk) k_segment_sort_walk<<<stiles, SG_THREADS, 0, ctx->stream>>>(ks, vs, counters, in.bits_lo, ko, vo, nullptr, counters + 5, tile_cnt, keep_all);
                else k_segment_sort<<<stiles, SG_THREADS, 0, ctx->stream>>>(ks, vs, counters, in.bits_lo, ko, vo, nullptr, counters + 5, tile_cnt, keep_all);
                CK(cudaGetLastError());
                if (tile_cnt) CKR((exclusive_scan<u64, u64>(ctx, ws, tile_cnt, tile_off, (u64)wtiles + 1)));
            } else {
                const u32 n_kept = h[0], h_long = h[5];
                unsigned char *flags;
                u64 *slot, *lk, *lk2, *lks;
                double *lv, *lv2, *lvs;
                u32 *lhist, *lcount;
                CKR(ws.get(&flags, n_kept));
                CKR(ws.get(&slot, (u64)n_kept + 1));
                CK(cudaMemsetAsync(counters + 5, 0, sizeof(u32), ctx->stream));
                ++ctx->launches;
                if (seg_shfl) k_segment_sort_shfl<<<stiles, SG_THREADS, 0, ctx->stream>>>(ks, vs, counters, in.bits_lo, ko, vo, flags, counters + 5);
                else if (seg_walk) k_segment_sort_walk<<<stiles, SG_THREADS, 0, ctx->stream>>>(ks, vs, counters, in.bits_lo, ko, vo, flags, counters + 5);
                else k_segment_sort<<<stiles, SG_THREADS, 0, ctx->stream>>>(ks, vs, counters, in.bits_lo, ko, vo, flags, counters + 5);
                CKR((exclusive_scan<unsigned char, u64>(ctx, ws, flags, slot, n_kept)));
                CKR(ws.get(&lk, h_long)); CKR(ws.get(&lv, h_long)); CKR(ws.get(&lk2, h_long)); CKR(ws.get(&lv2, h_long));
                CKR(ws.zeroed(&lhist, (u64)passes_full * RS_RADIX));
                CKR(ws.zeroed(&lcount, 8));
                CK(cudaMemcpyAsync(lcount, &h_long, sizeof(u32), cudaMemcpyHostToDevice, ctx->stream));
                ++ctx->launches, k_gather_flagged<<<grid_for(n_kept, 256, sgrid * 4), 256, 0, ctx->stream>>>(ks, vs, flags, slot, n_kept, lk, lv);
                ++ctx->launches, k_keys_hist<<<grid_for(h_long, 512, sgrid), 512, 0, ctx->stream>>>(lk, h_long, passes_full, lhist);
                ++ctx->launches, k_bucket_starts<<<passes_full, RS_RADIX, 0, ctx->stream>>>(lhist);
                CKR(run_radix_passes(ctx, ws, 1, passes_full, h_long, lcount, lhist, lk, lv, lk2, lv2, nullptr, &lks, &lvs, nullptr, nullptr));
                ++ctx->launches, k_scatter_flagged<<<grid_for(n_kept, 256, sgrid * 4), 256, 0, ctx->stream>>>(lks, lvs, flags, slot, n_kept, ko, vo);
                CK(cudaGetLastError());
            }
            ks = ko; vs = vo;
        }
        t1 = tm.mark();

        const bool rwarp = !fused && (tile_off != nullptr || rw_mode == 2);
        const u32 rtiles = rwarp ? wtiles / RW_WARPS : (u32)div_up(n, RK_TILE);
        ReduceArgs ra;
        memset(&ra, 0, sizeof ra);
        ra.keys = ks; ra.vals = vs; ra.n_ptr = counters; ra.bits_lo = in.bits_lo; ra.policy = job.policy;
        ra.out_hi = out_hi; ra.out_lo = out_lo; ra.out_val = out_val; ra.out_count = counters + 2;
        if (tile_off) ra.state = tile_off;
        else CKR(ws.zeroed(&ra.state, rwarp ? (u64)wtiles : (u64)rtiles));
        CKR(ws.zeroed(&ra.ticket, 1));
        ra.long_cap = n / RK_LONG_RUN + 1;
        CKR(ws.get(&ra.long_list, 2ull * ra.long_cap));
        ra.long_count = counters + 3;
        ra.row_start = row_start; ra.row_id = row_id; ra.row_count = counters + 4;
        if (fused) {
            ++ctx->launches, k_reduce_segsort<<<rtiles, RK_THREADS, sizeof(RfSmem), ctx->stream>>>(ra, counters + 5);
        } else {
            if (rwarp && tile_off) ++ctx->launches, k_reduce_warp<false><<<rtiles, RW_THREADS, 0, ctx->stream>>>(ra);
            else if (rwarp) ++ctx->launches, k_reduce_warp<true><<<rtiles, RW_THREADS, 0, ctx->stream>>>(ra);
            else ++ctx->launches, k_reduce_by_key<MODE_CONSOLIDATE><<<rtiles, RK_THREADS, 0, ctx->stream>>>(ra);
            if (job.policy == POLICY_ADD || job.policy == POLICY_REPLACE)
                ++ctx->launches, k_long_runs<<<(u32)ctx->sm_count * 4, 256, 0, ctx->stream>>>(ra);
        }
        CK(cudaGetLastError());
        t2 = tm.mark();

        CK(cudaMemcpyAsync(h, counters, sizeof h, cudaMemcpyDeviceToHost, ctx->stream));
        CK(cudaStreamSynchronize(ctx->stream));
        if (h[5] && !h[1] && attempt == 0 && seg) {
            fused = false;
            long_rows_fixed = true;
            CK(cudaMemsetAsync(counters + 2, 0, 3 * sizeof(u32), ctx->stream));
            continue;
        }
        break;
    }
    if (h[1]) return spb_fail(SPB_ERR_ARG, "Sparse index out of bounds (an index is negative or >= its extent)");
    *h_kept = h[0];
    *h_out = h[2];
    if (h_rows) *h_rows = h[4];
    if (st) {
        st->n_in = n; st->n_kept = h[0]; st->n_out = h[2];
        st->key_bits = key_bits; st->passes = passes; st->digit_bits = digit_bits;
        st->ms_sort = tm.ms(t0, t1); st->ms_reduce = tm.ms(t1, t2); st->ms_total = tm.ms(t0, t2);
        st->ms_pass = passes > 1 ? tm.ms(t_p0, t_passes) / (float)(passes - 1) : 0.f;
    }
    return 0;
}

static int consolidate_core(spb_ctx *ctx, const spb_coo *in, const int *so, const int *ref_so, int policy,
                            bool drop_zero, int zero_nan, spb_coo **out, spb_consolidate_stats *st,
                            i32 *ext_lo = nullptr, double *ext_val = nullptr) {
    if (in->n >= (1ull << 31)) return spb_fail(SPB_ERR_TOO_LARGE, "%llu entries: one array holds fewer than 2^31 (the reference's own cap, algorithm.hpp:419)", (ull)in->n);
    spb_coo *r = nullptr;
    if (ext_lo && ext_val && in->rank == 2) {
        CKR(coo_new(ctx, in->rank, in->shape, in->n, false, &r));
        r->owned = true;
        if (ctx->pool.alloc((void **)&r->idx[so[0]], (in->n ? in->n : 1) * sizeof(i32)) != cudaSuccess) {
            delete r;
            return spb_fail(SPB_ERR_CUDA, "out of device memory");
        }
        r->idx[so[1]] = ext_lo;
        r->val = ext_val;
    } else {
        CKR(coo_new(ctx, in->rank, in->shape, in->n, true, &r));
    }
    set_order(r, so);
    if (st) memset(st, 0, sizeof *st);
    if (in->n == 0) { *out = r; return SPB_OK; }
    const int d0 = so[0], d1 = in->rank > 1 ? so[1] : -1;
    SortJob job;
    memset(&job, 0, sizeof job);
    job.in.hi = in->idx[d0];
    job.in.lo = d1 >= 0 ? in->idx[d1] : nullptr;
    job.in.val = in->val;
    job.in.n = (u32)in->n;
    job.in.bits_lo = d1 >= 0 ? bits_for(in->shape[d1]) : 0;
    job.in.extent_hi = (u32)(in->shape[d0] > 0xffffffffull ? 0xffffffffu : in->shape[d0]);
    job.in.extent_lo = d1 >= 0 ? (u32)in->shape[d1] : 1u;
    job.in.drop_zero = drop_zero ? 1 : 0;
    job.in.drop_nan = (drop_zero && zero_nan) ? 1 : 0;
    const int r0 = ref_so[0], r1 = in->rank > 1 ? ref_so[1] : -1;
    job.in.ref_hi = in->idx[r0];
    job.in.ref_lo = r1 >= 0 ? in->idx[r1] : nullptr;
    job.in.ref_bits_lo = r1 >= 0 ? bits_for(in->shape[r1]) : 0;
    job.bits_hi = bits_for(in->shape[d0]);
    job.policy = policy;
    u32 kept = 0, nout = 0, nrows = 0;
    if (in->rank == 2) {
        const u64 cap = (in->n < in->shape[d0] ? in->n : in->shape[d0]) + 1;
        if (ctx->pool.alloc((void **)&r->row_start, cap * sizeof(u32)) != cudaSuccess ||
            ctx->pool.alloc((void **)&r->row_id, cap * sizeof(i32)) != cudaSuccess) {
            spb_coo_free(ctx, r);
            return spb_fail(SPB_ERR_CUDA, "out of device memory");
        }
    }
    int rc = sort_reduce(ctx, job, r->idx[d0], d1 >= 0 ? r->idx[d1] : nullptr, r->val, &kept, &nout, st,
                         r->row_start, r->row_id, &nrows);
    if (rc) { spb_coo_free(ctx, r); return rc; }
    r->n = nout;
    if (in->rank == 2) {
        r->nrows = nrows;
        r->rows_valid = true;
        if (nout == 0) { const u32 z = 0; cudaMemcpyAsync(r->row_start, &z, sizeof z, cudaMemcpyHostToDevice, ctx->stream); }
    }
    *out = r;
    return SPB_OK;
}

static int check_order(const spb_coo *a, const int *so, const char *what) {
    if (!so) return spb_fail(SPB_ERR_ARG, "%s: sort_order is null", what);
    for (int k = 0; k < a->rank; ++k)
        if (a->n && !a->idx[k]) return spb_fail(SPB_ERR_ARG, "%s: array is in compressed (pointer) form", what);
    bool seen[2] = {false, false};
    for (int k = 0; k < a->rank; ++k) {
        if (so[k] < 0 || so[k] >= a->rank || seen[so[k]])
            return spb_fail(SPB_ERR_ARG, "%s: sort_order is not a permutation of the dimensions", what);
        seen[so[k]] = true;
    }
    return 0;
}

struct RowIndex {
    u32 *start;
    i32 *id;
    u32 nrows;
};

static int build_row_index(spb_ctx *ctx, const spb_coo *a_const, RowIndex *ri) {
    spb_coo *a = const_cast<spb_coo *>(a_const);
    if (!a->rows_valid && a->n && !a->idx[a->sort_order[0]])
        return spb_fail(SPB_ERR_ARG, "array in compressed (pointer) form has no row list; use it as the B operand only");
    if (!a->rows_valid) {
        const u32 n = (u32)a->n;
        const i32 *hi = a->idx[a->sort_order[0]];
        Scratch ws(ctx);
        u32 *rs = nullptr;
        i32 *rid = nullptr;
        CK(ctx->pool.alloc((void **)&rs, ((u64)n + 1) * sizeof(u32)));
        if (ctx->pool.alloc((void **)&rid, ((u64)n + 1) * sizeof(i32)) != cudaSuccess) {
            ctx->pool.release(rs);
            return spb_fail(SPB_ERR_CUDA, "out of device memory (row list of %u entries)", n);
        }
        a->row_start = rs; a->row_id = rid;
        u32 *count, *ticket;
        u64 *state;
        const u32 tiles = (u32)div_up(n ? n : 1, RH_TILE);
        CKR(ws.zeroed(&count, 1));
        CKR(ws.zeroed(&ticket, 1));
        CKR(ws.zeroed(&state, tiles));
        if (n) ++ctx->launches, k_row_heads<<<tiles, RH_THREADS, 0, ctx->stream>>>(hi, n, a->row_start, a->row_id, count, state, ticket);
        ++ctx->launches, k_row_sentinel<<<1, 1, 0, ctx->stream>>>(a->row_start, count, n);
        CK(cudaGetLastError());
        CK(cudaMemcpyAsync(&a->nrows, count, sizeof(u32), cudaMemcpyDeviceToHost, ctx->stream));
        CK(cudaStreamSynchronize(ctx->stream));
        a->rows_valid = true;
    }
    ri->start = a->row_start;
    ri->id = a->row_id;
    ri->nrows = a->nrows;
    return 0;
}

template <typename InT, typename OutT>
static int exclusive_scan(spb_ctx *ctx, Scratch &ws, const InT *in, OutT *out, u64 n) {
    if (n == 0) { CK(cudaMemsetAsync(out, 0, sizeof(OutT), ctx->stream)); return 0; }
    const u32 tiles = (u32)div_up(n, SC_TILE);
    u64 *state;
    u32 *ticket;
    CKR(ws.zeroed(&state, tiles));
    CKR(ws.zeroed(&ticket, 1));
    ++ctx->launches, k_exclusive_scan<InT, OutT><<<tiles, SC_THREADS, 0, ctx->stream>>>(in, out, n, state, ticket);
    CK(cudaGetLastError());
    return 0;
}

static int build_dense_ptr(spb_ctx *ctx, const spb_coo *a_const, u64 extent, u32 **ptr_out) {
    spb_coo *a = const_cast<spb_coo *>(a_const);
    if (!a->dense_ptr) {
        RowIndex ri;
        CKR(build_row_index(ctx, a, &ri));
        CK(ctx->pool.alloc((void **)&a->dense_ptr, (extent + 2) * sizeof(u32)));
        Scratch ws(ctx);
        DpGap *gaps = nullptr;
        u32 *n_gaps = nullptr;
        if (ri.nrows && extent + 1 - ri.nrows >= DP_LONG_GAP) {
            CKR(ws.get(&gaps, (extent + 1) / DP_LONG_GAP + 1));
            CKR(ws.zeroed(&n_gaps, 1));
        }
        ++ctx->launches;
        if (ri.nrows) k_dense_ptr_from_rows<<<grid_for(ri.nrows, 256, (u32)ctx->sm_count * 16), 256, 0, ctx->stream>>>(ri.start, ri.id, ri.nrows, (u32)a->n, extent, a->dense_ptr, gaps, n_gaps);
        else k_fill_u32<<<grid_for(extent + 1, 256, (u32)ctx->sm_count * 16), 256, 0, ctx->stream>>>(a->dense_ptr, extent + 1, 0u);
        if (gaps) ++ctx->launches, k_fill_gaps<<<(u32)ctx->sm_count * 8, 256, 0, ctx->stream>>>(gaps, n_gaps, a->dense_ptr);
        CK(cudaGetLastError());
    }
    *ptr_out = a->dense_ptr;
    return 0;
}

static int densify(spb_ctx *ctx, Scratch &ws, const spb_coo *v, u64 dim, double **dense, unsigned char **mask, u32 *bad) {
    CKR(ws.zeroed(dense, dim));
    if (mask) CKR(ws.zeroed(mask, dim));
    if (v->n) ++ctx->launches, k_densify<<<grid_for(v->n, 256, 1u << 16), 256, 0, ctx->stream>>>(v->idx[0], v->val, v->n, dim, *dense, mask ? *mask : nullptr, bad);
    CK(cudaGetLastError());
    return 0;
}
static int bad_scale_vector() {
    return spb_fail(SPB_ERR_ARG, "a scale vector (or a vector operand flagged sorted) is not strictly ascending in its index: the "
                    "reference joins these as sorted lists without repeats (xiter.hpp:146, 201)");
}

static int esc_sort_reduce(spb_ctx *ctx, u64 *kA, double *vA, u32 count, int key_bits, int kbits,
                           const MMOperands &m, u32 row_lo, i32 *t_row, i32 *t_k, double *t_v, u32 *h_out) {
    Scratch ws(ctx);
    int passes = (key_bits + RS_RADIX_BITS - 1) / RS_RADIX_BITS;
    if (passes < 1) passes = 1;
    u32 *hist, *counters;
    CKR(ws.zeroed(&hist, (u64)passes * RS_RADIX));
    CKR(ws.zeroed(&counters, 8));
    CK(cudaMemcpyAsync(counters, &count, sizeof(u32), cudaMemcpyHostToDevice, ctx->stream));
    ++ctx->launches, k_keys_hist<<<grid_for(count, 512, (u32)ctx->sm_count * 4), 512, 0, ctx->stream>>>(kA, count, passes, hist);
    ++ctx->launches, k_bucket_starts<<<passes, RS_RADIX, 0, ctx->stream>>>(hist);
    u64 *kB, *ks;
    double *vB, *vs;
    CKR(ws.get(&kB, count));
    CKR(ws.get(&vB, count));
    {
        const u32 tiles = (u32)div_up(count, RS_TILE);
        u32 *lookback, *tickets;
        CKR(ws.zeroed(&lookback, (u64)passes * tiles * RS_RADIX));
        CKR(ws.zeroed(&tickets, (u64)passes));
        u64 *kin = kA, *kout = kB;
        double *vin = vA, *vout = vB;
        SortInput dummy;
        memset(&dummy, 0, sizeof dummy);
        for (int p = 0; p < passes; ++p) {
            PassArgs a;
            a.keys_in = kin; a.vals_in = vin; a.keys_out = kout; a.vals_out = vout;
            a.n_ptr = counters;
            a.bucket_start = hist + (u64)p * RS_RADIX;
            a.lookback = lookback + (u64)p * tiles * RS_RADIX;
            a.ticket = tickets + p;
            a.shift = p * RS_RADIX_BITS;
            a.rank_mode = 0;
        a.rank_mode = getenv("SPB_RANK_MODE") ? atoi(getenv("SPB_RANK_MODE")) : 0;
            ++ctx->launches;
            if (ctx->bulk_load) k_radix_pass<false, true><<<tiles, RS_THREADS, RS_SMEM_BYTES, ctx->stream>>>(a, dummy);
            else k_radix_pass<false><<<tiles, RS_THREADS, RS_SMEM_BYTES, ctx->stream>>>(a, dummy);
            u64 *tk = kin; kin = kout; kout = tk;
            double *tv = vin; vin = vout; vout = tv;
        }
        ks = kin; vs = vin;
        CK(cudaGetLastError());
    }
    const u32 rtiles = (u32)div_up(count, RK_TILE);
    ReduceArgs ra;
    memset(&ra, 0, sizeof ra);
    ra.keys = ks; ra.vals = vs; ra.n_ptr = counters; ra.bits_lo = kbits; ra.policy = POLICY_ADD;
    ra.out_hi = t_row; ra.out_lo = t_k; ra.out_val = t_v; ra.out_count = counters + 2;
    CKR(ws.zeroed(&ra.state, rtiles));
    CKR(ws.zeroed(&ra.ticket, 1));
    ra.row_ids = m.arow_id; ra.row_base = (i32)row_lo; ra.si = m.si; ra.sk = m.sk; ra.C = m.C;
    ++ctx->launches, k_reduce_by_key<MODE_ESC><<<rtiles, RK_THREADS, 0, ctx->stream>>>(ra);
    CK(cudaGetLastError());
    CK(cudaMemcpyAsync(h_out, counters + 2, sizeof(u32), cudaMemcpyDeviceToHost, ctx->stream));
    CK(cudaStreamSynchronize(ctx->stream));
    return 0;
}

struct EscChunk { i32 *row; i32 *k; double *v; u32 n; };

static size_t ballast_for_blocks(int blocks_per_sm, size_t static_smem) {
    if (blocks_per_sm <= 0) return 0;
    const size_t per = (size_t)(227 * 1024) / (size_t)blocks_per_sm;
    return per > static_smem + 1024 ? per - static_smem - 1024 : 0;
}
template <typename K> static int allow_ballast(K kernel) {
    static thread_local const void *done[16];
    static thread_local int n = 0;
    for (int i = 0; i < n; ++i) if (done[i] == (const void *)kernel) return 0;
    CK(cudaFuncSetAttribute(kernel, cudaFuncAttributeMaxDynamicSharedMemorySize, 200 * 1024));
    if (n < 16) done[n++] = (const void *)kernel;
    return 0;
}

struct PreScale {
    const double *sj;
    const unsigned char *sj_mask;
};

static int multiply_core(spb_ctx *ctx, double C, const spb_coo *si, const spb_coo *A, int a_row_dim,
                         const spb_coo *sj, const spb_coo *B, int b_inner_dim, const spb_coo *sk,
                         spb_coo *out, spb_mm_stats *st, Timer &tm, int t_begin, bool symbolic_only = false,
                         const PreScale *pre = nullptr) {
    Scratch ws(ctx);
    const int a_in = 1 - a_row_dim, b_col = 1 - b_inner_dim;
    const u64 m_rows = A->shape[a_row_dim], n_inner = A->shape[a_in], n_cols = B->shape[b_col];
    MMOperands m;
    memset(&m, 0, sizeof m);
    m.C = C;
    m.debug = getenv("SPB_MERGE_DEBUG") ? atoi(getenv("SPB_MERGE_DEBUG")) : 0;
    m.a_j = A->idx[a_in]; m.a_val = A->val; m.nnz_a = (u32)A->n;
    RowIndex ri;
    CKR(build_row_index(ctx, A, &ri));
    m.arow_id = ri.id; m.arow_start = ri.start; m.nrows = ri.nrows;
    u32 *bptr;
    CKR(build_dense_ptr(ctx, B, n_inner, &bptr));
    m.bptr = bptr; m.b_k = B->idx[b_col]; m.b_val = B->val;
    double *d;
    unsigned char *mask;
    u32 *bad_vec;
    CKR(ws.zeroed(&bad_vec, 1));
    if (si) { CKR(densify(ctx, ws, si, m_rows, &d, nullptr, bad_vec)); m.si = d; }
    if (pre) { m.sj = pre->sj; m.sj_mask = pre->sj_mask; }
    else if (sj) { CKR(densify(ctx, ws, sj, n_inner, &d, &mask, bad_vec)); m.sj = d; m.sj_mask = mask; }
    if (sk) { CKR(densify(ctx, ws, sk, n_cols, &d, nullptr, bad_vec)); m.sk = d; }
    const int t_prep = tm.mark();
    double h0 = now_ms();
    if (tracing()) fprintf(stderr, "[spb] mm: prepare done (host), alloc so far %.2f ms\n", g_alloc_ms);

    const u32 nrows = m.nrows;
    u32 *row_cnt;
    u64 *ent_off = nullptr, *esc_f = nullptr, *esc_off, *c_ptr;
    unsigned char *row_cls;
    ull *stats;
    CKR(ws.get(&row_cls, nrows));
    CKR(ws.zeroed(&row_cnt, (u64)nrows + 1));
    ull *mstats;
    CKR(ws.zeroed(&stats, 8));
    CKR(ws.zeroed(&mstats, (u64)MC_STRIPES * 8));
    const u32 cap = (u32)ctx->sm_count * 32;
    {
        const double avg_a_len = nrows ? (double)m.nnz_a / (double)nrows : 0.0;
        const double avg_b = n_inner ? (double)B->n / (double)n_inner : 0.0;
        const u64 cap_out = (u64)nrows * 16;
        const bool want = !symbolic_only && nrows && avg_a_len * avg_b <= 40.0 && (A->max_row_len == 0 || A->max_row_len <= (u32)MERGE_MAX_LISTS) &&
                          cap_out < (1ull << 31) && cap_out * 16 <= (48ull << 30) &&
                          getenv("SPB_MERGE_ONEPASS") && atoi(getenv("SPB_MERGE_ONEPASS")) != 0;
        if (want) {
            spb_coo *Am1 = const_cast<spb_coo *>(A);
            if (!Am1->max_row_len) {
                u32 *mx;
                CKR(ws.zeroed(&mx, 1));
                ++ctx->launches, k_row_maxlen<<<grid_for(nrows, 256, cap), 256, 0, ctx->stream>>>(m.arow_start, nrows, mx);
                CK(cudaMemcpyAsync(&Am1->max_row_len, mx, sizeof(u32), cudaMemcpyDeviceToHost, ctx->stream));
                CK(cudaStreamSynchronize(ctx->stream));
            }
            const u32 ml = A->max_row_len;
            if (ml <= (u32)MERGE_MAX_LISTS) {
                const u32 g = (u32)div_up(nrows, MR_THREADS);
                u64 *state;
                u32 *tk;
                ull *o1;
                i32 *ci = nullptr, *ck = nullptr;
                double *cv = nullptr;
                CKR(ws.zeroed(&state, (u64)g * (MR_THREADS / 32)));
                CKR(ws.zeroed(&tk, 2));
                CKR(ws.zeroed(&o1, 8 + (u64)MC_STRIPES * 8));
                if (ctx->pool.alloc((void **)&ci, cap_out * sizeof(i32)) != cudaSuccess || ctx->pool.alloc((void **)&ck, cap_out * sizeof(i32)) != cudaSuccess ||
                    ctx->pool.alloc((void **)&cv, cap_out * sizeof(double)) != cudaSuccess) {
                    cudaGetLastError();
                    ctx->pool.release(ci); ctx->pool.release(ck); ctx->pool.release(cv);
                } else {
                    ++ctx->launches;
                    if (ml <= 2) k_merge_onepass<2><<<g, MR_THREADS, 0, ctx->stream>>>(m, ctx->merge_max_products, state, tk, tk + 1, o1, ci, ck, cv);
                    else if (ml <= 4) k_merge_onepass<4><<<g, MR_THREADS, 0, ctx->stream>>>(m, ctx->merge_max_products, state, tk, tk + 1, o1, ci, ck, cv);
                    else if (ml <= 6) k_merge_onepass<6><<<g, MR_THREADS, 0, ctx->stream>>>(m, ctx->merge_max_products, state, tk, tk + 1, o1, ci, ck, cv);
                    else k_merge_onepass<8><<<g, MR_THREADS, 0, ctx->stream>>>(m, ctx->merge_max_products, state, tk, tk + 1, o1, ci, ck, cv);
                    CK(cudaGetLastError());
                    const int t_one = tm.mark();
                    ull h_o[8 + MC_STRIPES * 8];
                    u32 h_tk[2], h_badv = 0;
                    CK(cudaMemcpyAsync(h_o, o1, sizeof h_o, cudaMemcpyDeviceToHost, ctx->stream));
                    CK(cudaMemcpyAsync(h_tk, tk, sizeof h_tk, cudaMemcpyDeviceToHost, ctx->stream));
                    CK(cudaMemcpyAsync(&h_badv, bad_vec, sizeof h_badv, cudaMemcpyDeviceToHost, ctx->stream));
                    CK(cudaStreamSynchronize(ctx->stream));
                    if (h_badv) { ctx->pool.release(ci); ctx->pool.release(ck); ctx->pool.release(cv); return bad_scale_vector(); }
                    if (!h_tk[1]) {
                        ull F1 = 0, rows1 = 0;
                        for (int sx = 0; sx < MC_STRIPES; ++sx) { F1 += h_o[8 + sx * 8]; rows1 += h_o[8 + sx * 8 + 1]; }
                        out->idx[0] = ci; out->idx[1] = ck; out->val = cv;
                        out->owned = true;
                        out->n = h_o[0];
                        if (st) {
                            st->products = F1; st->rows_merge = rows1; st->nnz_a = A->n; st->nnz_b = B->n; st->rows_a = nrows; st->nnz_c = h_o[0];
                            st->ms_prepare = tm.ms(t_begin, t_prep);
                            st->ms_symbolic = 0.f;
                            st->ms_numeric = tm.ms(t_prep, t_one);
                            st->ms_merge_numeric = st->ms_numeric;
                            st->ms_total = tm.ms(t_begin, t_one);
                        }
                        return SPB_OK;
                    }
                    ctx->pool.release(ci); ctx->pool.release(ck); ctx->pool.release(cv);
                }
            }
        }
    }

    const double avg_b_len = n_inner ? (double)B->n / (double)n_inner : 0.0;
    spb_coo *Am = const_cast<spb_coo *>(A);
    const bool maxlen_up_front = !Am->max_row_len && nrows && (avg_b_len > 16.0 || getenv("SPB_MERGE_NL_COUNT"));
// ... 1322 lines not shown
```

Before: 42.88 billion.

## Write segment-sort output as split hi/lo index arrays and hand buffers to result

The segment sort kernels now write row and column indices as separate i32 arrays straight into output buffers instead of packed u64 keys, and the reduce stage reads split keys through a templated accessor. When the reduction turns out to be an identity, the sorted buffers are handed over to the result instead of being copied. The fused reduce-segsort kernel and the shuffle variant are removed. The aim is to cut key bytes written and read and to skip a final copy, at the cost of more plumbing and two 4-byte loads per key comparison in the long-run search.

```diff
diff --git a/spsparse_b200/csrc/radix_sort.cuh b/spsparse_b200/csrc/radix_sort.cuh
--- a/spsparse_b200/csrc/radix_sort.cuh
+++ b/spsparse_b200/csrc/radix_sort.cuh
@@ -398,7 +398,7 @@
 
 constexpr int SG_CNT_SHIFT = 8;
 __global__ void __launch_bounds__(SG_THREADS, 5) k_segment_sort(const u64 *__restrict__ keys_in, const double *__restrict__ vals_in,
-                                                                const u32 *n_ptr, int bits_lo, u64 *keys_out, double *vals_out,
+                                                                const u32 *n_ptr, int bits_lo, i32 *hi_out, i32 *lo_out, double *vals_out,
                                                                 unsigned char *flags, u32 *long_count, u64 *tile_cnt = nullptr,
                                                                 int keep_all = 0) {
     constexpr int W = SG_TILE + 2 * SEG_MAX;
@@ -531,7 +531,9 @@
         const u64 g = wbase + (u64)k * 32 + lane;
         if (g < n) {
             const u64 dst = (u64)((i64)g + shift_by[k]);
-            keys_out[dst] = s_key[SEG_MAX + warp * 256 + k * 32 + lane];
+            const u64 key = s_key[SEG_MAX + warp * 256 + k * 32 + lane];
+            hi_out[dst] = (i32)(key >> bits_lo);
+            lo_out[dst] = (i32)(key & lo_mask);
             vals_out[dst] = v[k];
         }
     }
@@ -545,7 +547,7 @@
 #endif
 constexpr int SGW_UNROLL = SGW_UNROLL_N;
 __global__ void __launch_bounds__(SG_THREADS, 6) k_segment_sort_walk(const u64 *__restrict__ keys_in, const double *__restrict__ vals_in,
-                                                             const u32 *n_ptr, int bits_lo, u64 *keys_out, double *vals_out,
+                                                             const u32 *n_ptr, int bits_lo, i32 *hi_out, i32 *lo_out, double *vals_out,
                                                              unsigned char *flags, u32 *long_count, u64 *tile_cnt = nullptr,
                                                              int keep_all = 0) {
     __shared__ u32 s_row[SG_TILE + 2 * SEG_MAX];
@@ -607,7 +609,8 @@
                 head = keep_all || same == 0;
                 rhead = before == 0;
             }
-            keys_out[dst] = ((u64)row << bits_lo) | col;
+            hi_out[dst] = (i32)row;
+            lo_out[dst] = (i32)col;
             vals_out[dst] = v[k];
             if (flags) flags[g] = is_long;
             n_long += is_long;
@@ -631,122 +634,20 @@
     if (n_long && lane == 0) atomicAdd(long_count, n_long);
 }
 
-constexpr int SGS_ROW = 5;
-constexpr int SGS_H = SGS_ROW - 1;
-constexpr int SGS_STEP = 32 - 2 * SGS_H;
-constexpr int SGS_STEPS = (256 + SGS_STEP - 1) / SGS_STEP;
-__global__ void __launch_bounds__(SG_THREADS, 6) k_segment_sort_shfl(const u64 *__restrict__ keys_in, const double *__restrict__ vals_in,
-                                                                    const u32 *n_ptr, int bits_lo, u64 *keys_out, double *vals_out,
-                                                                    unsigned char *flags, u32 *long_count, u64 *tile_cnt = nullptr,
-                                                                    int keep_all = 0) {
-    __shared__ u32 s_row[SG_TILE + 2 * SEG_MAX];
-    __shared__ u32 s_col[SG_TILE + 2 * SEG_MAX];
-    __shared__ double s_val[SG_TILE];
-    const u32 n = *n_ptr;
-    const u64 base = (u64)blockIdx.x * SG_TILE;
-    if (base >= n) return;
-    const u32 tid = threadIdx.x, lane = tid & 31, warp = tid >> 5;
-    const u32 lo_mask = bits_lo >= 32 ? 0xffffffffu : (1u << bits_lo) - 1u;
-    for (u32 q = tid; q < SG_TILE + 2 * SEG_MAX; q += SG_THREADS) {
-        const i64 g = (i64)base + (i64)q - SEG_MAX;
-        u32 row = 0xffffffffu, col = 0;
-        if (g >= 0 && g < (i64)n) {
-            const u64 key = ld_stream_u64(keys_in + g);
-            row = (u32)(key >> bits_lo);
-            col = (u32)key & lo_mask;
-        }
-        s_row[q] = row;
-        s_col[q] = col;
-    }
-#pragma unroll
-    for (int k = 0; k < SG_IPT; ++k) {
-        const u32 e = (u32)k * SG_THREADS + tid;
-        const u64 g = base + e;
-        s_val[e] = g < n ? ld_stream_f64(vals_in + g) : 0.0;
-    }
-    __syncthreads();
-    const u64 wbase = base + (u64)warp * 256;
-    u32 n_long = 0;
-    u32 cnt_at = 0, cnt_before = 0, cnt_after = 0;
-    for (int t = 0; t < SGS_STEPS; ++t) {
-        const i32 e = t * SGS_STEP + (i32)lane - SGS_H;
-        const u32 q = (u32)(SEG_MAX + (i32)warp * 256 + e);
-        const u64 g = wbase + (u64)(i64)e;
-        const bool mine = lane >= (u32)SGS_H && lane < (u32)(32 - SGS_H) && e < 256 && g < n;
-        const u32 row = s_row[q], col = s_col[q];
-        const u32 hb = __ballot_sync(SPB_FULL_MASK, s_row[q - 1] != row);
-        const u32 tail = __shfl_sync(SPB_FULL_MASK, (u32)(s_row[q + 1] != row), 31);
-        const u64 z = ~((u64)hb | ((u64)tail << 32)) & 0x1ffffffffull;
-        u64 run = z;
-#pragma unroll
-        for (int d = 1; d < SGS_ROW; ++d) run &= z >> d;
-        u32 b = 0, f = 0, before = 0, same = 0;
-        if (run == 0) {
-#pragma unroll
-            for (int d = 1; d < SGS_ROW; ++d) {
-                const u32 ru = __shfl_up_sync(SPB_FULL_MASK, row, d), cu = __shfl_up_sync(SPB_FULL_MASK, col, d);
-                const u32 rd = __shfl_down_sync(SPB_FULL_MASK, row, d), cd = __shfl_down_sync(SPB_FULL_MASK, col, d);
-                const bool up = lane >= (u32)d && ru == row, dn = lane + d < 32u && rd == row;
-                b += up;
-                before += (up && cu <= col) + (dn && cd < col);
-                same += up && cu == col;
-                f += dn;
-            }
-        } else if (mine) {
-            if (s_row[q - SEG_MAX] == row || s_row[q + SEG_MAX] == row) b = f = (u32)SEG_MAX;
-            else {
-                for (b = 0; b < (u32)SEG_MAX; ++b) {
-                    if (s_row[q - 1 - b] != row) break;
-                    const u32 c = s_col[q - 1 - b];
-                    before += c <= col;
-                    same += c == col;
-                }
-                for (f = 0; f < (u32)SEG_MAX; ++f) {
-                    if (s_row[q + 1 + f] != row) break;
-                    before += s_col[q + 1 + f] < col;
-                }
-            }
-        }
-        if (mine) {
-            const bool is_long = b == (u32)SEG_MAX || f == (u32)SEG_MAX || b + f + 1 > (u32)SEG_MAX;
-            u64 dst = g;
-            bool head = true, rhead = false;
-            if (!is_long) {
-                dst = g - b + before;
-                head = keep_all || same == 0;
-                rhead = before == 0;
-            }
-            keys_out[dst] = ((u64)row << bits_lo) | col;
-            vals_out[dst] = s_val[warp * 256 + (u32)e];
-            if (flags) flags[g] = is_long;
-            n_long += is_long;
-            const u32 inc = (head ? 1u : 0u) | (rhead ? 0x10000u : 0u);
-            if (dst < wbase) cnt_before += inc;
-            else if (dst >= wbase + 256) cnt_after += inc;
-            else cnt_at += inc;
-        }
-    }
-    if (tile_cnt) {
-        const u32 a0 = __reduce_add_sync(SPB_FULL_MASK, cnt_at), a1 = __reduce_add_sync(SPB_FULL_MASK, cnt_before),
-                  a2 = __reduce_add_sync(SPB_FULL_MASK, cnt_after);
-        if (lane == 0) {
-            u64 *t = tile_cnt + (wbase >> SG_CNT_SHIFT);
-            if (a0) atomicAdd((ull *)t, (ull)(a0 & 0xffffu) | ((ull)(a0 >> 16) << 31));
-            if (a1) atomicAdd((ull *)(t - 1), (ull)(a1 & 0xffffu) | ((ull)(a1 >> 16) << 31));
-            if (a2) atomicAdd((ull *)(t + 1), (ull)(a2 & 0xffffu) | ((ull)(a2 >> 16) << 31));
-        }
-    }
-    n_long = __reduce_add_sync(SPB_FULL_MASK, n_long);
-    if (n_long && lane == 0) atomicAdd(long_count, n_long);
-}
-
 __global__ void k_gather_flagged(const u64 *__restrict__ keys, const double *__restrict__ vals, const unsigned char *__restrict__ flags,
                                  const u64 *__restrict__ slot, u32 n, u64 *k_out, double *v_out) {
     for (u64 e = (u64)blockIdx.x * blockDim.x + threadIdx.x; e < n; e += (u64)gridDim.x * blockDim.x)
         if (flags[e]) { k_out[slot[e]] = keys[e]; v_out[slot[e]] = vals[e]; }
 }
 __global__ void k_scatter_flagged(const u64 *__restrict__ k_sorted, const double *__restrict__ v_sorted,
-                                  const unsigned char *__restrict__ flags, const u64 *__restrict__ slot, u32 n, u64 *keys, double *vals) {
+                                  const unsigned char *__restrict__ flags, const u64 *__restrict__ slot, u32 n, int bits_lo,
+                                  i32 *hi, i32 *lo, double *vals) {
+    const u64 lo_mask = (1ull << bits_lo) - 1;
     for (u64 e = (u64)blockIdx.x * blockDim.x + threadIdx.x; e < n; e += (u64)gridDim.x * blockDim.x)
-        if (flags[e]) { keys[e] = k_sorted[slot[e]]; vals[e] = v_sorted[slot[e]]; }
-}
+        if (flags[e]) {
+            const u64 key = k_sorted[slot[e]];
+            hi[e] = (i32)(key >> bits_lo);
+            lo[e] = (i32)(key & lo_mask);
+            vals[e] = v_sorted[slot[e]];
+        }
+}
diff --git a/spsparse_b200/csrc/reduce_by_key.cuh b/spsparse_b200/csrc/reduce_by_key.cuh
--- a/spsparse_b200/csrc/reduce_by_key.cuh
+++ b/spsparse_b200/csrc/reduce_by_key.cuh
@@ -15,6 +15,8 @@
 
 struct ReduceArgs {
     const u64 *keys;
+    const i32 *in_hi;
+    const i32 *in_lo;
     const double *vals;
     const u32 *n_ptr;
     int bits_lo;
@@ -31,6 +33,8 @@
     u32 *row_start;
     i32 *row_id;
     u32 *row_count;
+    const u32 *seg_long;
+    u32 *identity;
     const i32 *row_ids;
     i32 row_base;
     const double *si;
@@ -39,6 +43,12 @@
 };
 
 __device__ __forceinline__ u32 rk_phys(u32 L) { return L + (L >> 3); }
+
+template <bool SPLIT>
+__device__ __forceinline__ u64 ra_key(const ReduceArgs &a, u64 i) {
+    if (SPLIT) return ((u64)(u32)a.in_hi[i] << a.bits_lo) | (u32)a.in_lo[i];
+    return a.keys[i];
+}
 constexpr int RK_SLOTS = RK_TILE + 2 + ((RK_TILE + 2) >> 3) + 1;
 
 #ifndef RK_MIN_BLOCKS
@@ -218,6 +228,7 @@
     }
 }
 
+template <bool SPLIT>
 __global__ void __launch_bounds__(256) k_long_runs(ReduceArgs a) {
     const u32 n = *a.n_ptr;
     u32 cnt = *a.long_count;
@@ -226,19 +237,19 @@
     const u32 warps = gridDim.x * (blockDim.x >> 5);
     for (u32 t = blockIdx.x * (blockDim.x >> 5) + (threadIdx.x >> 5); t < cnt; t += warps) {
         const u32 slot = a.long_list[2 * t], start = a.long_list[2 * t + 1];
-        const u64 key = a.keys[start];
+        const u64 key = ra_key<SPLIT>(a, start);
         u32 lo = start + 1, step = RK_LONG_RUN;
         u32 hi = n;
         for (;;) {
             const u64 probe = (u64)lo + step;
             if (probe >= n) break;
-            if (a.keys[probe] > key) { hi = (u32)probe; break; }
+            if (ra_key<SPLIT>(a, probe) > key) { hi = (u32)probe; break; }
             lo = (u32)probe + 1;
             step *= 2;
         }
         while (lo < hi) {
             const u32 mid = lo + (hi - lo) / 2;
-            if (a.keys[mid] <= key) lo = mid + 1; else hi = mid;
+            if (ra_key<SPLIT>(a, mid) <= key) lo = mid + 1; else hi = mid;
         }
         const u32 end = lo;
         double r;
diff --git a/spsparse_b200/csrc/reduce_segsort.cuh b/spsparse_b200/csrc/reduce_segsort.cuh
--- a/spsparse_b200/csrc/reduce_segsort.cuh
+++ /dev/null
@@ -1,194 +0,0 @@
-#pragma once
-#include "radix_sort.cuh"
-#include "reduce_by_key.cuh"
-
-constexpr int RF_H = SEG_MAX;
-constexpr int RF_W = RK_TILE + 2 * RF_H;
-constexpr int RF_ITS = (RF_W + RK_THREADS - 1) / RK_THREADS;
-constexpr int RF_SORTED = RK_TILE + RF_H + 1;
-constexpr int RF_SLOTS = RF_SORTED + (RF_SORTED >> 3) + 1;
-
-struct RfSmem {
-    u64 raw[RF_W];
-    u64 keys[RF_SLOTS];
-    double vals[RF_SLOTS];
-    u64 warp[RK_WARPS];
-    u64 excl;
-    u32 tile;
-};
-
-__global__ void __launch_bounds__(RK_THREADS, 4) k_reduce_segsort(ReduceArgs a, u32 *seg_long) {
-    extern __shared__ __align__(16) unsigned char rf_smem[];
-    RfSmem &s = *reinterpret_cast<RfSmem *>(rf_smem);
-    const u32 tid = threadIdx.x, lane = tid & 31, warp = tid >> 5;
-    const bool want_rows = a.row_start != nullptr;
-    if (tid == 0) s.tile = atomicAdd(a.ticket, 1u);
-    __syncthreads();
-    const u32 tile = s.tile;
-    const u32 n = *a.n_ptr;
-    const u64 base = (u64)tile * RK_TILE;
-    if (base >= n) return;
-    const u32 tile_n = (n - base < (u64)RK_TILE) ? (u32)(n - base) : (u32)RK_TILE;
-
-    double v[RF_ITS];
-#pragma unroll
-    for (int k = 0; k < RF_ITS; ++k) {
-        const u32 q = (u32)k * RK_THREADS + tid;
-        const i64 g = (i64)base + (i64)q - RF_H;
-        const bool in = q < (u32)RF_W && g >= 0 && g < (i64)n;
-        if (q < (u32)RF_W) s.raw[q] = in ? ld_stream_u64(a.keys + g) : ~0ull;
-        v[k] = in ? ld_stream_f64(a.vals + g) : 0.0;
-    }
-    __syncthreads();
-
-    const u64 lo_mask = (1ull << a.bits_lo) - 1;
-    u32 n_long = 0;
-#pragma unroll
-    for (int k = 0; k < RF_ITS; ++k) {
-        const u32 q = (u32)k * RK_THREADS + tid;
-        if (q >= (u32)RF_W) continue;
-        const u64 key = s.raw[q];
-        if (key == ~0ull) continue;
-        const u64 row = key >> a.bits_lo, col = key & lo_mask;
-        u32 b = 0, f = 0, before = 0;
-        bool cut = false;
-        for (; b < (u32)SEG_MAX; ++b) {
-            if (q < 1 + b) { cut = true; break; }
-            const u64 kk = s.raw[q - 1 - b];
-            if ((kk >> a.bits_lo) != row) break;
-            before += (kk & lo_mask) <= col;
-        }
-        for (; f < (u32)SEG_MAX; ++f) {
-            if (q + 1 + f >= (u32)RF_W) { cut = true; break; }
-            const u64 kk = s.raw[q + 1 + f];
-            if ((kk >> a.bits_lo) != row) break;
-            before += (kk & lo_mask) < col;
-        }
-        const bool is_long = b == (u32)SEG_MAX || f == (u32)SEG_MAX || b + f + 1 > (u32)SEG_MAX;
-        if (q >= (u32)RF_H && q < (u32)(RF_H + RK_TILE)) n_long += is_long;
-        const u32 place = (cut || is_long) ? q : q - b + before;
-        if (place + 1 >= (u32)RF_H && place + 1 < (u32)(RF_H + RF_SORTED)) {
-            const u32 L = place + 1 - (u32)RF_H;
-            s.keys[rk_phys(L)] = key;
-            s.vals[rk_phys(L)] = v[k];
-        }
-    }
-    n_long = __reduce_add_sync(SPB_FULL_MASK, n_long);
-    if (n_long && lane == 0) atomicAdd(seg_long, n_long);
-    __syncthreads();
-
-    const u32 first = tid * RK_IPT;
-    const u32 mine = first < tile_n ? (tile_n - first < (u32)RK_IPT ? tile_n - first : (u32)RK_IPT) : 0;
-    u64 key[RK_IPT];
-    double acc[RK_IPT];
-    u32 head_bits = 0, rhead_bits = 0;
-    if (mine) {
-        const u64 prev = s.keys[rk_phys(first)];
-#pragma unroll
-        for (int j = 0; j < RK_IPT; ++j) {
-            key[j] = s.keys[rk_phys(first + j + 1)];
-            acc[j] = s.vals[rk_phys(first + j + 1)];
-        }
-        int cur = -1;
-#pragma unroll
-        for (int j = 0; j < RK_IPT; ++j) {
-            if ((u32)j < mine) {
-                const u64 before = j ? key[j - 1] : prev;
-                const bool head = (a.policy == POLICY_KEEP_ALL) || (base + first + j == 0) || (key[j] != before);
-                if (head) {
-                    head_bits |= 1u << j;
-                    if (want_rows && ((base + first + j == 0) || (key[j] >> a.bits_lo) != (before >> a.bits_lo)))
-                        rhead_bits |= 1u << j;
-                    cur = j;
-                } else if (cur >= 0) {
-                    const double vj = acc[j];
-#pragma unroll
-                    for (int h = 0; h < RK_IPT; ++h)
-                        if (h == cur) {
-                            if (a.policy == POLICY_ADD) acc[h] = __dadd_rn(acc[h], vj);
-                            else if (a.policy == POLICY_REPLACE) acc[h] = vj;
-                        }
-                }
-            }
-        }
-        if (cur >= 0 && mine == (u32)RK_IPT && (a.policy == POLICY_ADD || a.policy == POLICY_REPLACE)) {
-            const u64 k0 = key[RK_IPT - 1];
-            double sum = 0.0;
-#pragma unroll
-            for (int h = 0; h < RK_IPT; ++h) if (h == cur) sum = acc[h];
-            u64 q = base + first + RK_IPT;
-            while (q < n) {
-                const u32 L = (u32)(q - base) + 1;
-                if (L >= (u32)RF_SORTED) break;
-                if (s.keys[rk_phys(L)] != k0) break;
-                const double vq = s.vals[rk_phys(L)];
-                if (a.policy == POLICY_ADD) sum = __dadd_rn(sum, vq); else sum = vq;
-                ++q;
-            }
-#pragma unroll
-            for (int h = 0; h < RK_IPT; ++h) if (h == cur) acc[h] = sum;
-        }
-    }
-    const u32 emit_bits = head_bits;
-    const u64 my = (u64)__popc(emit_bits) | ((u64)__popc(rhead_bits) << 32);
-    const u64 incl = warp_incl_scan(my);
-    if (lane == 31) s.warp[warp] = incl;
-    __syncthreads();
-    u64 wbefore = 0, total = 0;
-#pragma unroll
-    for (int w = 0; w < RK_WARPS; ++w) {
-        const u64 t = s.warp[w];
-        if ((u32)w < warp) wbefore += t;
-        total += t;
-    }
-    const u64 before_me = wbefore + incl - my;
-    const u32 tile_out = (u32)(total & 0xffffffffull);
-    if (warp == 0) {
-        const u64 packed = (total & 0xffffffffull) | ((total >> 32) << 31);
-        const u64 excl0 = lookback_exclusive(a.state, tile, packed);
-        if (lane == 0) {
-            s.excl = excl0;
-            if (base + RK_TILE >= n) {
-                const u64 fin = excl0 + packed;
-                const u32 n_out = (u32)(fin & 0x7fffffffull), n_rows = (u32)(fin >> 31);
-                *a.out_count = n_out;
-                if (want_rows) { *a.row_count = n_rows; a.row_start[n_rows] = n_out; }
-            }
-        }
-    }
-    {
-        u32 slot = (u32)(before_me & 0xffffffffull);
-#pragma unroll
-        for (int j = 0; j < RK_IPT; ++j) {
-            if ((emit_bits >> j) & 1u) {
-                s.keys[slot] = key[j];
-                s.vals[slot] = acc[j];
-                ++slot;
-            }
-        }
-    }
-    __syncthreads();
-    const u64 excl_rows = s.excl >> 31;
-    const u64 excl = s.excl & 0x7fffffffull;
-    if (rhead_bits) {
-        u32 slot = (u32)(before_me & 0xffffffffull);
-        u64 rslot = excl_rows + (before_me >> 32);
-#pragma unroll
-        for (int j = 0; j < RK_IPT; ++j) {
-            if ((emit_bits >> j) & 1u) {
-                if ((rhead_bits >> j) & 1u) {
-                    a.row_start[rslot] = (u32)(excl + slot);
-                    a.row_id[rslot] = (i32)(key[j] >> a.bits_lo);
-                    ++rslot;
-                }
-                ++slot;
-            }
-        }
-    }
-    for (u32 t = tid; t < tile_out; t += RK_THREADS) {
-        const u64 k = s.keys[t];
-        a.out_hi[excl + t] = (i32)(k >> a.bits_lo);
-        if (a.out_lo) a.out_lo[excl + t] = (i32)(k & lo_mask);
-        a.out_val[excl + t] = s.vals[t];
-    }
-}
diff --git a/spsparse_b200/csrc/reduce_warp.cuh b/spsparse_b200/csrc/reduce_warp.cuh
--- a/spsparse_b200/csrc/reduce_warp.cuh
+++ b/spsparse_b200/csrc/reduce_warp.cuh
@@ -10,8 +10,9 @@
 #define RW_MIN_BLOCKS 4
 #endif
 
-template <bool LOOKBACK>
+template <bool LOOKBACK, bool SPLIT>
 __global__ void __launch_bounds__(RW_THREADS, RW_MIN_BLOCKS) k_reduce_warp(ReduceArgs a) {
+    static_assert(LOOKBACK || SPLIT, "the tile offsets from head counts exist only after the in-row sort");
     __shared__ u64 s_keys[RW_WARPS][RW_SLOTS];
     __shared__ double s_vals[RW_WARPS][RW_SLOTS];
     __shared__ u32 s_ticket;
@@ -24,22 +25,76 @@
     }
     const u32 n = *a.n_ptr;
     const u64 base = (u64)tile * RW_TILE;
+    const bool want_rows = a.row_start != nullptr;
+    if (!LOOKBACK) {
+        const u64 fin = a.state[gridDim.x * RW_WARPS];
+        if (*a.seg_long == 0 && (u32)(fin & 0x7fffffffull) == n) {
+            if (tile == 0 && lane == 0) {
+                *a.identity = 1u;
+                *a.out_count = n;
+                if (want_rows) { *a.row_count = (u32)(fin >> 31); a.row_start[fin >> 31] = n; }
+            }
+            if (base >= n || !want_rows) return;
+            const u32 tile_n = (n - base < (u64)RW_TILE) ? (u32)(n - base) : (u32)RW_TILE;
+            const u32 first = lane * RW_IPT;
+            const u32 mine = first < tile_n ? (tile_n - first < (u32)RW_IPT ? tile_n - first : (u32)RW_IPT) : 0;
+            i32 hi[RW_IPT];
+            if (tile_n == (u32)RW_TILE && (((uintptr_t)a.in_hi) & 15u) == 0) {
+                const int4 *hp = reinterpret_cast<const int4 *>(a.in_hi + base + first);
+                const int4 t0 = __ldg(hp), t1 = __ldg(hp + 1);
+                hi[0] = t0.x; hi[1] = t0.y; hi[2] = t0.z; hi[3] = t0.w; hi[4] = t1.x; hi[5] = t1.y; hi[6] = t1.z; hi[7] = t1.w;
+            } else {
+#pragma unroll
+                for (int j = 0; j < RW_IPT; ++j) hi[j] = (u32)j < mine ? a.in_hi[base + first + j] : 0;
+            }
+            i32 prev = __shfl_up_sync(SPB_FULL_MASK, hi[RW_IPT - 1], 1);
+            if (lane == 0) prev = base ? a.in_hi[base - 1] : -1;
+            u32 rhead_bits = 0;
+#pragma unroll
+            for (int j = 0; j < RW_IPT; ++j)
+                if ((u32)j < mine && hi[j] != (j ? hi[j - 1] : prev)) rhead_bits |= 1u << j;
+            const u32 my = __popc(rhead_bits);
+            const u32 incl = (u32)warp_incl_scan((u64)my);
+            u64 rslot = (a.state[tile] >> 31) + incl - my;
+#pragma unroll
+            for (int j = 0; j < RW_IPT; ++j)
+                if ((rhead_bits >> j) & 1u) {
+                    a.row_start[rslot] = (u32)(base + first + j);
+                    a.row_id[rslot] = hi[j];
+                    ++rslot;
+                }
+            return;
+        }
+    }
     if (base >= n) return;
     const u32 tile_n = (n - base < (u64)RW_TILE) ? (u32)(n - base) : (u32)RW_TILE;
-    const bool want_rows = a.row_start != nullptr;
     const u32 first = lane * RW_IPT;
     const u32 mine = first < tile_n ? (tile_n - first < (u32)RW_IPT ? tile_n - first : (u32)RW_IPT) : 0;
 
     u64 key[RW_IPT];
     double acc[RW_IPT];
-    if (tile_n == (u32)RW_TILE && ((((uintptr_t)a.keys) | ((uintptr_t)a.vals)) & 15u) == 0) {
-        const ulonglong2 *kp = reinterpret_cast<const ulonglong2 *>(a.keys + base + first);
+    const uintptr_t in_addr = SPLIT ? (((uintptr_t)a.in_hi) | ((uintptr_t)a.in_lo)) : (uintptr_t)a.keys;
+    if (tile_n == (u32)RW_TILE && ((in_addr | ((uintptr_t)a.vals)) & 15u) == 0) {
+        if (SPLIT) {
+            const int4 *hp = reinterpret_cast<const int4 *>(a.in_hi + base + first);
+            const int4 *lp = reinterpret_cast<const int4 *>(a.in_lo + base + first);
+#pragma unroll
+            for (int j = 0; j < RW_IPT / 4; ++j) {
+                const int4 h = __ldg(hp + j), l = __ldg(lp + j);
+                key[4 * j + 0] = ((u64)(u32)h.x << a.bits_lo) | (u32)l.x;
+                key[4 * j + 1] = ((u64)(u32)h.y << a.bits_lo) | (u32)l.y;
+                key[4 * j + 2] = ((u64)(u32)h.z << a.bits_lo) | (u32)l.z;
+                key[4 * j + 3] = ((u64)(u32)h.w << a.bits_lo) | (u32)l.w;
+            }
+        } else {
+            const ulonglong2 *kp = reinterpret_cast<const ulonglong2 *>(a.keys + base + first);
+#pragma unroll
+            for (int j = 0; j < RW_IPT / 2; ++j) {
+                const ulonglong2 t = __ldg(kp + j);
+                key[2 * j] = t.x; key[2 * j + 1] = t.y;
+            }
+        }
         const double2 *vp = reinterpret_cast<const double2 *>(a.vals + base + first);
-#pragma unroll
-        for (int j = 0; j < RW_IPT / 2; ++j) {
-            const ulonglong2 t = __ldg(kp + j);
-            key[2 * j] = t.x; key[2 * j + 1] = t.y;
-        }
 #pragma unroll
         for (int j = 0; j < RW_IPT / 2; ++j) {
             const double2 t = __ldg(vp + j);
@@ -49,14 +104,14 @@
 #pragma unroll
         for (int j = 0; j < RW_IPT; ++j) {
             key[j] = 0; acc[j] = 0.0;
-            if ((u32)j < mine) { key[j] = a.keys[base + first + j]; acc[j] = a.vals[base + first + j]; }
+            if ((u32)j < mine) { key[j] = ra_key<SPLIT>(a, base + first + j); acc[j] = a.vals[base + first + j]; }
         }
     }
     u64 prev = __shfl_up_sync(SPB_FULL_MASK, key[RW_IPT - 1], 1);
-    if (lane == 0) prev = base ? a.keys[base - 1] : 0;
+    if (lane == 0) prev = base ? ra_key<SPLIT>(a, base - 1) : 0;
     u64 next = __shfl_down_sync(SPB_FULL_MASK, key[0], 1);
     const bool more = base + first + RW_IPT < n;
-    if (lane == 31 && more) next = a.keys[base + RW_TILE];
+    if (lane == 31 && more) next = ra_key<SPLIT>(a, base + RW_TILE);
 
     u32 head_bits = 0, rhead_bits = 0, defer_bits = 0;
     if (mine) {
@@ -91,7 +146,7 @@
             u64 q = base + first + RW_IPT;
             u32 steps = 0;
             while (q < n) {
-                if (a.keys[q] != k0) break;
+                if (ra_key<SPLIT>(a, q) != k0) break;
                 const double vq = a.vals[q];
                 if (a.policy == POLICY_ADD) sum = __dadd_rn(sum, vq); else sum = vq;
                 ++q;
diff --git a/spsparse_b200/csrc/spb_api.cu b/spsparse_b200/csrc/spb_api.cu
--- a/spsparse_b200/csrc/spb_api.cu
+++ b/spsparse_b200/csrc/spb_api.cu
@@ -17,7 +17,6 @@
 #include "radix_sort.cuh"
 #include "radix_sort9.cuh"
 #include "reduce_by_key.cuh"
-#include "reduce_segsort.cuh"
 #include "reduce_warp.cuh"
 #include "scan.cuh"
 #include "spgemm.cuh"
@@ -320,7 +319,6 @@
     CK(cudaDeviceGetAttribute(&c->sm_count, cudaDevAttrMultiProcessorCount, device));
     CK(cudaFuncSetAttribute(k_radix_pass<true>, cudaFuncAttributeMaxDynamicSharedMemorySize, (int)RS_SMEM_BYTES));
     CK(cudaFuncSetAttribute(k_radix_pass<false>, cudaFuncAttributeMaxDynamicSharedMemorySize, (int)RS_SMEM_BYTES));
-    CK(cudaFuncSetAttribute(k_reduce_segsort, cudaFuncAttributeMaxDynamicSharedMemorySize, (int)sizeof(RfSmem)));
     CK(cudaFuncSetAttribute(k_radix_pass9<true>, cudaFuncAttributeMaxDynamicSharedMemorySize, (int)R9_SMEM_BYTES));
     CK(cudaFuncSetAttribute(k_radix_pass9<false>, cudaFuncAttributeMaxDynamicSharedMemorySize, (int)R9_SMEM_BYTES));
     CK(cudaFuncSetAttribute(k_radix_pass<false, true>, cudaFuncAttributeMaxDynamicSharedMemorySize, (int)RS_SMEM_BYTES));
@@ -631,9 +629,11 @@
     return 0;
 }
 
+static inline u64 split_lo_offset(u64 n) { return (n + 3) & ~3ull; }
+
 static int sort_reduce(spb_ctx *ctx, const SortJob &job, i32 *out_hi, i32 *out_lo, double *out_val,
-                       u32 *h_kept, u32 *h_out, spb_consolidate_stats *st, u32 *row_start = nullptr,
-                       i32 *row_id = nullptr, u32 *h_rows = nullptr) {
+                       u32 *h_kept, u32 *h_out, spb_consolidate_stats *st, u32 *row_start, i32 *row_id, u32 *h_rows,
+                       i32 **moved_idx, double **moved_val) {
     const SortInput &in = job.in;
     const u32 n = in.n;
     const int key_bits = job.bits_hi + in.bits_lo;
@@ -646,7 +646,6 @@
     const bool seg_short = (double)n <= 16.0 * (double)in.extent_hi && n >= (1u << 23);
     const char *walk_env = getenv("SPB_SEGMENT_WALK");
     const bool seg_walk = walk_env ? atoi(walk_env) != 0 : (double)n <= 6.0 * (double)in.extent_hi;
-    const bool seg_shfl = walk_env && atoi(walk_env) == 2;
     const bool seg = in.bits_lo > 0 && passes_full - passes_row >= 2 &&
                      (seg_env ? atoi(seg_env) != 0 : seg_short);
     const int cover_bits = seg ? job.bits_hi : key_bits;
@@ -693,41 +692,40 @@
 
     u64 *kA, *kB = nullptr, *ks;
     double *vA, *vB = nullptr, *vs;
-    CKR(ws.get(&kA, n));
+    const u64 nk = split_lo_offset(n);
+    CKR(ws.get(&kA, nk));
     CKR(ws.get(&vA, n));
-    if (passes > 1 || seg) { CKR(ws.get(&kB, n)); CKR(ws.get(&vB, n)); }
+    if (passes > 1 || seg) { CKR(ws.get(&kB, nk)); CKR(ws.get(&vB, n)); }
     int t_p0 = t0;
     CKR(run_radix_passes(ctx, ws, 0, passes, n, counters, hist, kA, vA, kB, vB, &in0, &ks, &vs, &tm, &t_p0, shift0, digit_bits));
     const int t_passes = tm.mark();
-    const char *fused_env = getenv("SPB_FUSED_REDUCE");
-    bool fused = seg && seg_walk && fused_env && atoi(fused_env) != 0;
-    u32 h[6];
+    u32 h[7];
     int t1 = t_passes, t2 = t_passes;
     u64 *const ks_rows = ks;
     double *const vs_rows = vs;
+    u64 *const ko = (ks == kA) ? kB : kA;
+    double *const vo = (vs == vA) ? vB : vA;
+    i32 *const red_hi = seg ? (i32 *)ko : out_hi;
+    i32 *const red_lo = seg ? (i32 *)ko + nk : out_lo;
+    double *const red_val = seg ? vo : out_val;
     bool long_rows_fixed = false;
     const int rw_mode = getenv("SPB_REDUCE_WARP") ? atoi(getenv("SPB_REDUCE_WARP")) : 1;
     const u32 wtiles = (u32)div_up(div_up(n ? n : 1, RW_TILE), RW_WARPS) * RW_WARPS;
     for (int attempt = 0;; ++attempt) {
         ks = ks_rows; vs = vs_rows;
-        u64 *ko = (ks == kA) ? kB : kA;
-        double *vo = (vs == vA) ? vB : vA;
         const u32 stiles = (u32)div_up(n, SG_TILE);
         u64 *tile_off = nullptr;
-        if (seg && !fused) {
+        if (seg) {
             if (!long_rows_fixed) {
-                u64 *tile_cnt = nullptr;
-                if (rw_mode == 1) {
-                    CKR(ws.zeroed(&tile_cnt, (u64)wtiles + 2));
-                    CKR(ws.get(&tile_off, (u64)wtiles + 2));
-                }
+                u64 *tile_cnt;
+                CKR(ws.zeroed(&tile_cnt, (u64)wtiles + 2));
+                CKR(ws.get(&tile_off, (u64)wtiles + 2));
                 const int keep_all = job.policy == POLICY_KEEP_ALL;
                 ++ctx->launches;
-                if (seg_shfl) k_segment_sort_shfl<<<stiles, SG_THREADS, 0, ctx->stream>>>(ks, vs, counters, in.bits_lo, ko, vo, nullptr, counters + 5, tile_cnt, keep_all);
-                else if (seg_walk) k_segment_sort_walk<<<stiles, SG_THREADS, 0, ctx->stream>>>(ks, vs, counters, in.bits_lo, ko, vo, nullptr, counters + 5, tile_cnt, keep_all);
-                else k_segment_sort<<<stiles, SG_THREADS, 0, ctx->stream>>>(ks, vs, counters, in.bits_lo, ko, vo, nullptr, counters + 5, tile_cnt, keep_all);
+                if (seg_walk) k_segment_sort_walk<<<stiles, SG_THREADS, 0, ctx->stream>>>(ks, vs, counters, in.bits_lo, out_hi, out_lo, out_val, nullptr, counters + 5, tile_cnt, keep_all);
+                else k_segment_sort<<<stiles, SG_THREADS, 0, ctx->stream>>>(ks, vs, counters, in.bits_lo, out_hi, out_lo, out_val, nullptr, counters + 5, tile_cnt, keep_all);
                 CK(cudaGetLastError());
-                if (tile_cnt) CKR((exclusive_scan<u64, u64>(ctx, ws, tile_cnt, tile_off, (u64)wtiles + 1)));
+                CKR((exclusive_scan<u64, u64>(ctx, ws, tile_cnt, tile_off, (u64)wtiles + 1)));
             } else {
                 const u32 n_kept = h[0], h_long = h[5];
                 unsigned char *flags;
@@ -738,9 +736,8 @@
                 CKR(ws.get(&slot, (u64)n_kept + 1));
                 CK(cudaMemsetAsync(counters + 5, 0, sizeof(u32), ctx->stream));
                 ++ctx->launches;
-                if (seg_shfl) k_segment_sort_shfl<<<stiles, SG_THREADS, 0, ctx->stream>>>(ks, vs, counters, in.bits_lo, ko, vo, flags, counters + 5);
-                else if (seg_walk) k_segment_sort_walk<<<stiles, SG_THREADS, 0, ctx->stream>>>(ks, vs, counters, in.bits_lo, ko, vo, flags, counters + 5);
-                else k_segment_sort<<<stiles, SG_THREADS, 0, ctx->stream>>>(ks, vs, counters, in.bits_lo, ko, vo, flags, counters + 5);
+                if (seg_walk) k_segment_sort_walk<<<stiles, SG_THREADS, 0, ctx->stream>>>(ks, vs, counters, in.bits_lo, out_hi, out_lo, out_val, flags, counters + 5);
+                else k_segment_sort<<<stiles, SG_THREADS, 0, ctx->stream>>>(ks, vs, counters, in.bits_lo, out_hi, out_lo, out_val, flags, counters + 5);
                 CKR((exclusive_scan<unsigned char, u64>(ctx, ws, flags, slot, n_kept)));
                 CKR(ws.get(&lk, h_long)); CKR(ws.get(&lv, h_long)); CKR(ws.get(&lk2, h_long)); CKR(ws.get(&lv2, h_long));
                 CKR(ws.zeroed(&lhist, (u64)passes_full * RS_RADIX));
@@ -750,19 +747,20 @@
                 ++ctx->launches, k_keys_hist<<<grid_for(h_long, 512, sgrid), 512, 0, ctx->stream>>>(lk, h_long, passes_full, lhist);
                 ++ctx->launches, k_bucket_starts<<<passes_full, RS_RADIX, 0, ctx->stream>>>(lhist);
                 CKR(run_radix_passes(ctx, ws, 1, passes_full, h_long, lcount, lhist, lk, lv, lk2, lv2, nullptr, &lks, &lvs, nullptr, nullptr));
-                ++ctx->launches, k_scatter_flagged<<<grid_for(n_kept, 256, sgrid * 4), 256, 0, ctx->stream>>>(lks, lvs, flags, slot, n_kept, ko, vo);
+                ++ctx->launches, k_scatter_flagged<<<grid_for(n_kept, 256, sgrid * 4), 256, 0, ctx->stream>>>(lks, lvs, flags, slot, n_kept, in.bits_lo, out_hi, out_lo, out_val);
                 CK(cudaGetLastError());
             }
-            ks = ko; vs = vo;
         }
         t1 = tm.mark();
 
-        const bool rwarp = !fused && (tile_off != nullptr || rw_mode == 2);
+        const bool rwarp = seg || rw_mode == 2;
         const u32 rtiles = rwarp ? wtiles / RW_WARPS : (u32)div_up(n, RK_TILE);
         ReduceArgs ra;
         memset(&ra, 0, sizeof ra);
-        ra.keys = ks; ra.vals = vs; ra.n_ptr = counters; ra.bits_lo = in.bits_lo; ra.policy = job.policy;
-        ra.out_hi = out_hi; ra.out_lo = out_lo; ra.out_val = out_val; ra.out_count = counters + 2;
+        ra.n_ptr = counters; ra.bits_lo = in.bits_lo; ra.policy = job.policy;
+        if (seg) { ra.in_hi = out_hi; ra.in_lo = out_lo; ra.vals = out_val; ra.seg_long = counters + 5; ra.identity = counters + 6; }
+        else { ra.keys = ks; ra.vals = vs; }
+        ra.out_hi = red_hi; ra.out_lo = red_lo; ra.out_val = red_val; ra.out_count = counters + 2;
         if (tile_off) ra.state = tile_off;
         else CKR(ws.zeroed(&ra.state, rwarp ? (u64)wtiles : (u64)rtiles));
         CKR(ws.zeroed(&ra.ticket, 1));
@@ -770,14 +768,15 @@
         CKR(ws.get(&ra.long_list, 2ull * ra.long_cap));
         ra.long_count = counters + 3;
         ra.row_start = row_start; ra.row_id = row_id; ra.row_count = counters + 4;
-        if (fused) {
-            ++ctx->launches, k_reduce_segsort<<<rtiles, RK_THREADS, sizeof(RfSmem), ctx->stream>>>(ra, counters + 5);
-        } else {
-            if (rwarp && tile_off) ++ctx->launches, k_reduce_warp<false><<<rtiles, RW_THREADS, 0, ctx->stream>>>(ra);
-            else if (rwarp) ++ctx->launches, k_reduce_warp<true><<<rtiles, RW_THREADS, 0, ctx->stream>>>(ra);
-            else ++ctx->launches, k_reduce_by_key<MODE_CONSOLIDATE><<<rtiles, RK_THREADS, 0, ctx->stream>>>(ra);
-            if (job.policy == POLICY_ADD || job.policy == POLICY_REPLACE)
-                ++ctx->launches, k_long_runs<<<(u32)ctx->sm_count * 4, 256, 0, ctx->stream>>>(ra);
+        ++ctx->launches;
+        if (tile_off) k_reduce_warp<false, true><<<rtiles, RW_THREADS, 0, ctx->stream>>>(ra);
+        else if (seg) k_reduce_warp<true, true><<<rtiles, RW_THREADS, 0, ctx->stream>>>(ra);
+        else if (rwarp) k_reduce_warp<true, false><<<rtiles, RW_THREADS, 0, ctx->stream>>>(ra);
+        else k_reduce_by_key<MODE_CONSOLIDATE><<<rtiles, RK_THREADS, 0, ctx->stream>>>(ra);
+        if (job.policy == POLICY_ADD || job.policy == POLICY_REPLACE) {
+            ++ctx->launches;
+            if (seg) k_long_runs<true><<<(u32)ctx->sm_count * 4, 256, 0, ctx->stream>>>(ra);
+            else k_long_runs<false><<<(u32)ctx->sm_count * 4, 256, 0, ctx->stream>>>(ra);
         }
         CK(cudaGetLastError());
         t2 = tm.mark();
@@ -785,14 +784,20 @@
         CK(cudaMemcpyAsync(h, counters, sizeof h, cudaMemcpyDeviceToHost, ctx->stream));
         CK(cudaStreamSynchronize(ctx->stream));
         if (h[5] && !h[1] && attempt == 0 && seg) {
-            fused = false;
             long_rows_fixed = true;
             CK(cudaMemsetAsync(counters + 2, 0, 3 * sizeof(u32), ctx->stream));
             continue;
         }
         break;
     }
+    *moved_idx = nullptr;
+    *moved_val = nullptr;
     if (h[1]) return spb_fail(SPB_ERR_ARG, "Sparse index out of bounds (an index is negative or >= its extent)");
+    if (seg && !h[6]) {
+        ws.keep(ko); ws.keep(vo);
+        *moved_idx = (i32 *)ko;
+        *moved_val = vo;
+    }
     *h_kept = h[0];
     *h_out = h[2];
     if (h_rows) *h_rows = h[4];
@@ -819,6 +824,21 @@
         }
         r->idx[so[1]] = ext_lo;
         r->val = ext_val;
+    } else if (in->rank == 2 && in->n) {
+        CKR(coo_new(ctx, in->rank, in->shape, in->n, false, &r));
+        r->owned = true;
+        i32 *idx = nullptr;
+        if (ctx->pool.alloc((void **)&idx, 2 * split_lo_offset(in->n) * sizeof(i32)) != cudaSuccess) {
+            delete r;
+            return spb_fail(SPB_ERR_CUDA, "out of device memory");
+        }
+        if (ctx->pool.alloc((void **)&r->val, in->n * sizeof(double)) != cudaSuccess) {
+            ctx->pool.release(idx);
+            delete r;
+            return spb_fail(SPB_ERR_CUDA, "out of device memory");
+        }
+        r->idx[so[0]] = idx;
+        r->idx[so[1]] = idx + split_lo_offset(in->n);
     } else {
         CKR(coo_new(ctx, in->rank, in->shape, in->n, true, &r));
     }
@@ -852,9 +872,27 @@
             return spb_fail(SPB_ERR_CUDA, "out of device memory");
         }
     }
+    i32 *moved_idx;
+    double *moved_val;
     int rc = sort_reduce(ctx, job, r->idx[d0], d1 >= 0 ? r->idx[d1] : nullptr, r->val, &kept, &nout, st,
-                         r->row_start, r->row_id, &nrows);
+                         r->row_start, r->row_id, &nrows, &moved_idx, &moved_val);
     if (rc) { spb_coo_free(ctx, r); return rc; }
+    if (moved_idx) {
+        const u64 lo_off = split_lo_offset(in->n);
+        if (r->idx[d1] == ext_lo) {
+            CK(cudaMemcpyAsync(r->idx[d0], moved_idx, (size_t)nout * sizeof(i32), cudaMemcpyDeviceToDevice, ctx->stream));
+            CK(cudaMemcpyAsync(ext_lo, moved_idx + lo_off, (size_t)nout * sizeof(i32), cudaMemcpyDeviceToDevice, ctx->stream));
+            CK(cudaMemcpyAsync(ext_val, moved_val, (size_t)nout * sizeof(double), cudaMemcpyDeviceToDevice, ctx->stream));
+            ctx->pool.release(moved_idx);
+            ctx->pool.release(moved_val);
+        } else {
+            ctx->pool.release(r->idx[d0]);
+            ctx->pool.release(r->val);
+            r->idx[d0] = moved_idx;
+            r->idx[d1] = moved_idx + lo_off;
+            r->val = moved_val;
+        }
+    }
     r->n = nout;
     if (in->rank == 2) {
         r->nrows = nrows;
```

Measured after the change: 46.16 billion, median of 6. +7.6%, better.
